# srendle/libfm

Hardware: NVIDIA H100
Metric: MovieLens-1M-shaped examples/sec at k=8, SGD (higher is better)
Workload: dtype f32

## Files before the change

include/fmb200.h:

```cpp
#ifndef FMB200_H_
#define FMB200_H_

#include <stdint.h>

#ifdef __cplusplus
extern "C" {
#endif

typedef struct fmb200_ctx fmb200_ctx;

#define FMB200_TASK_REGRESSION 0
#define FMB200_TASK_CLASSIFICATION 1

#define FMB200_MODE_INORDER 0
#define FMB200_MODE_HOGWILD 1

#define FMB200_MODE_ORDERED 2

#define FMB200_MAX_SLOTS 8
#define FMB200_MAX_PEERS 16
#define FMB200_IPC_HANDLE_BYTES 64

int fmb200_create(fmb200_ctx** out, int device, uint32_t n_attr, int num_factor, int use_w0,
                  int use_w);
void fmb200_destroy(fmb200_ctx* ctx);
const char* fmb200_last_error(void);

int fmb200_set_hparams(fmb200_ctx* ctx, int task, double learn_rate, double reg0, double regw,
                       double regv, double min_target, double max_target);
int fmb200_set_mode(fmb200_ctx* ctx, int mode);

int fmb200_upload_data(fmb200_ctx* ctx, int slot, uint64_t n_rows, uint64_t nnz,
                       const uint64_t* row_ptr, const uint32_t* col, const float* val,
                       const float* target);
int fmb200_upload_data_async(fmb200_ctx* ctx, int slot, uint64_t n_rows, uint64_t nnz,
                             const uint64_t* row_ptr, const uint32_t* col, const float* val,
                             const float* target);
int fmb200_upload_data_aos(fmb200_ctx* ctx, int slot, uint64_t n_rows, const void* rows,
                           const float* target);
int fmb200_upload_onehot(fmb200_ctx* ctx, int slot, uint64_t n_rows, uint32_t nnz_per_row,
                         const uint32_t* ids, const float* target);
int fmb200_upload_onehot_async(fmb200_ctx* ctx, int slot, uint64_t n_rows, uint32_t nnz_per_row,
                               const uint32_t* ids, const float* target);
int fmb200_free_data(fmb200_ctx* ctx, int slot);

int fmb200_host_alloc(void** out, uint64_t bytes);
int fmb200_host_free(void* p);

int fmb200_set_params(fmb200_ctx* ctx, double w0, const double* w, const double* v_factor_major);
int fmb200_get_params(fmb200_ctx* ctx, double* w0, double* w, double* v_factor_major);

int fmb200_sgd_epoch(fmb200_ctx* ctx, int slot, double* device_seconds);
int fmb200_sgd_epoch_async(fmb200_ctx* ctx, int slot);
int fmb200_sync(fmb200_ctx* ctx);

int fmb200_evaluate(fmb200_ctx* ctx, int slot, double* sum_sq_err, double* sum_abs_err,
                    uint64_t* n_correct);

int fmb200_predict(fmb200_ctx* ctx, int slot, int transform, double* out);

int fmb200_mcmc_eterms(fmb200_ctx* ctx, int slot, double* e_out);

int fmb200_mcmc_begin(fmb200_ctx* ctx, int train_slot, int test_slot, int do_sample, int do_multilevel,
                      uint32_t n_groups, const uint32_t* attr_group, const uint32_t* attr_per_group, double reg0,
                      const double* w_lambda, const double* v_lambda);
int fmb200_mcmc_iteration(fmb200_ctx* ctx, double* train_metric, uint32_t* counters);
int fmb200_mcmc_get_hyper(fmb200_ctx* ctx, double* alpha, double* w_mu, double* w_lambda, double* v_mu,
                          double* v_lambda);
int fmb200_mcmc_get_pred(fmb200_ctx* ctx, double* pred_this, double* pred_sum_all, double* pred_sum_all_but5);
int fmb200_mcmc_runs(fmb200_ctx* ctx, uint32_t* n_runs);

int fmb200_sgda_begin(fmb200_ctx* ctx, uint32_t n_groups, const uint32_t* attr_group);
int fmb200_sgda_epoch(fmb200_ctx* ctx, int train_slot, int val_slot, int lambda_steps, double* device_seconds);
int fmb200_sgda_get_reg(fmb200_ctx* ctx, double* reg_w, double* reg_v);

int fmb200_params_device(fmb200_ctx* ctx, void** device_ptr, uint64_t* n_floats);
int fmb200_scale_params(fmb200_ctx* ctx, double factor);
int fmb200_params_layout(fmb200_ctx* ctx, uint64_t* off_w, int* ws, uint64_t* off_v, int* kp);
int fmb200_stream(fmb200_ctx* ctx, void** cuda_stream);

int fmb200_peer_export(fmb200_ctx* ctx, void* handle );
int fmb200_peer_attach_ipc(fmb200_ctx* ctx, int world, int rank, const void* handles );
int fmb200_peer_attach_local(fmb200_ctx* ctx, int world, int rank, fmb200_ctx* const* contexts);
int fmb200_allreduce_mean(fmb200_ctx* ctx);
int fmb200_allreduce_meanfield(fmb200_ctx* ctx);
int fmb200_peer_barrier(fmb200_ctx* ctx);

int fmb200_download_data(fmb200_ctx* ctx, int slot, uint64_t* n_rows, uint64_t* nnz, uint64_t* row_ptr,
                         uint32_t* col, float* val, float* target);
int fmb200_kernel_launches(fmb200_ctx* ctx, uint64_t* count);
int fmb200_last_epoch_config(fmb200_ctx* ctx, int* lanes_per_row, int* slots, int* rows_per_tile,
                             int* grid, int* block, int* smem_bytes, int* damp);
int fmb200_set_tuning(fmb200_ctx* ctx, int ctas_per_sm, int rows_per_tile, int threads, int damp,
                      int variant);
int fmb200_ordered_index(fmb200_ctx* ctx, int slot, uint32_t* link ,
                         uint32_t* rowdep );

#ifdef __cplusplus
}
#endif
#endif
```

libfm_b200/_capi.py:

```python
from __future__ import annotations

import ctypes as C
import os

_HERE = os.path.dirname(os.path.abspath(__file__))
LIB_PATH = os.environ.get("FMB200_LIB") or os.path.join(_HERE, "lib", "libfmb200.so")

_u64p = C.POINTER(C.c_uint64)
_u32p = C.POINTER(C.c_uint32)
_f32p = C.POINTER(C.c_float)
_f64p = C.POINTER(C.c_double)
_intp = C.POINTER(C.c_int)
_ctx = C.c_void_p

SYMBOLS = {
    "fmb200_create": (C.c_int, [C.POINTER(_ctx), C.c_int, C.c_uint32, C.c_int, C.c_int, C.c_int]),
    "fmb200_destroy": (None, [_ctx]),
    "fmb200_last_error": (C.c_char_p, []),
    "fmb200_set_hparams": (C.c_int, [_ctx, C.c_int] + [C.c_double] * 6),
    "fmb200_set_mode": (C.c_int, [_ctx, C.c_int]),
    "fmb200_upload_data": (C.c_int, [_ctx, C.c_int, C.c_uint64, C.c_uint64, _u64p, _u32p, _f32p, _f32p]),
    "fmb200_upload_data_async": (C.c_int, [_ctx, C.c_int, C.c_uint64, C.c_uint64, _u64p, _u32p, _f32p, _f32p]),
    "fmb200_upload_data_aos": (C.c_int, [_ctx, C.c_int, C.c_uint64, C.c_void_p, _f32p]),
    "fmb200_upload_onehot": (C.c_int, [_ctx, C.c_int, C.c_uint64, C.c_uint32, _u32p, _f32p]),
    "fmb200_upload_onehot_async": (C.c_int, [_ctx, C.c_int, C.c_uint64, C.c_uint32, _u32p, _f32p]),
    "fmb200_free_data": (C.c_int, [_ctx, C.c_int]),
    "fmb200_host_alloc": (C.c_int, [C.POINTER(C.c_void_p), C.c_uint64]),
    "fmb200_host_free": (C.c_int, [C.c_void_p]),
    "fmb200_set_params": (C.c_int, [_ctx, C.c_double, _f64p, _f64p]),
    "fmb200_get_params": (C.c_int, [_ctx, _f64p, _f64p, _f64p]),
    "fmb200_sgd_epoch": (C.c_int, [_ctx, C.c_int, _f64p]),
    "fmb200_sgd_epoch_async": (C.c_int, [_ctx, C.c_int]),
    "fmb200_sync": (C.c_int, [_ctx]),
    "fmb200_evaluate": (C.c_int, [_ctx, C.c_int, _f64p, _f64p, _u64p]),
    "fmb200_predict": (C.c_int, [_ctx, C.c_int, C.c_int, _f64p]),
    "fmb200_sgda_begin": (C.c_int, [_ctx, C.c_uint32, _u32p]),
    "fmb200_sgda_epoch": (C.c_int, [_ctx, C.c_int, C.c_int, C.c_int, _f64p]),
    "fmb200_sgda_get_reg": (C.c_int, [_ctx, _f64p, _f64p]),
    "fmb200_mcmc_eterms": (C.c_int, [_ctx, C.c_int, _f64p]),
    "fmb200_mcmc_begin": (C.c_int, [_ctx, C.c_int, C.c_int, C.c_int, C.c_int, C.c_uint32, _u32p, _u32p, C.c_double,
                                    _f64p, _f64p]),
    "fmb200_mcmc_iteration": (C.c_int, [_ctx, _f64p, _u32p]),
    "fmb200_mcmc_get_hyper": (C.c_int, [_ctx] + [_f64p] * 5),
    "fmb200_mcmc_get_pred": (C.c_int, [_ctx] + [_f64p] * 3),
    "fmb200_mcmc_runs": (C.c_int, [_ctx, _u32p]),
    "fmb200_params_device": (C.c_int, [_ctx, C.POINTER(C.c_void_p), _u64p]),
    "fmb200_scale_params": (C.c_int, [_ctx, C.c_double]),
    "fmb200_params_layout": (C.c_int, [_ctx, _u64p, _intp, _u64p, _intp]),
    "fmb200_stream": (C.c_int, [_ctx, C.POINTER(C.c_void_p)]),
    "fmb200_peer_export": (C.c_int, [_ctx, C.c_void_p]),
    "fmb200_peer_attach_ipc": (C.c_int, [_ctx, C.c_int, C.c_int, C.c_void_p]),
    "fmb200_peer_attach_local": (C.c_int, [_ctx, C.c_int, C.c_int, C.POINTER(_ctx)]),
    "fmb200_allreduce_mean": (C.c_int, [_ctx]),
    "fmb200_allreduce_meanfield": (C.c_int, [_ctx]),
    "fmb200_peer_barrier": (C.c_int, [_ctx]),
    "fmb200_download_data": (C.c_int, [_ctx, C.c_int, _u64p, _u64p, _u64p, _u32p, _f32p, _f32p]),
    "fmb200_kernel_launches": (C.c_int, [_ctx, _u64p]),
    "fmb200_last_epoch_config": (C.c_int, [_ctx] + [_intp] * 7),
    "fmb200_set_tuning": (C.c_int, [_ctx, C.c_int, C.c_int, C.c_int, C.c_int, C.c_int]),
    "fmb200_ordered_index": (C.c_int, [_ctx, C.c_int, _u32p, _u32p]),
}

_lib = None


def load() -> C.CDLL:
    global _lib
    if _lib is None:
        if not os.path.exists(LIB_PATH):
            raise ImportError(
                f"{LIB_PATH} is missing: build it with `python -m libfm_b200.build` "
                "(libfm_b200 has no CPU fallback)")
        lib = C.CDLL(LIB_PATH)
        for name, (res, args) in SYMBOLS.items():
            fn = getattr(lib, name)
            fn.restype = res
            fn.argtypes = args
        _lib = lib
    return _lib
```

libfm_b200/build.py:

```python
from __future__ import annotations

import concurrent.futures as cf
import os
import shutil
import subprocess
import sys

HERE = os.path.dirname(os.path.abspath(__file__))
ROOT = os.path.dirname(HERE)
CSRC = os.path.join(HERE, "csrc")
HOST = os.path.join(HERE, "host")
LIBDIR = os.path.join(HERE, "lib")
OBJDIR = os.path.join(ROOT, "build", "obj")
BINDIR = os.path.join(ROOT, "bin")

NVCC = os.environ.get("NVCC") or shutil.which("nvcc") or "/usr/local/cuda/bin/nvcc"
ARCH = ["-gencode", "arch=compute_90a,code=sm_90a"]
COMMON = ["-O3", "-std=c++17", "-lineinfo", "-Xcompiler", "-fPIC", "-Xptxas", "-v",
          "-I", os.path.join(ROOT, "include")]

CU_SOURCES = {
    "fm_context.cu": [],
    "fm_hogwild.cu": [],
    "fm_rowlane.cu": [],
    "fm_peer.cu": [],
    "fm_predict.cu": [],
    "fm_inorder.cu": ["--fmad=false"],
    "fm_ordered.cu": [],
    "fm_upload.cu": [],
    "fm_mcmc.cu": ["--fmad=false"],
}
CU_HEADERS = ["fm_device.cuh", "fm_rowgroup.cuh", "fm_hogwild_common.cuh", "fmb200_internal.h",
              "fm_inorder_wavefront.cuh", "fm_ordered.cuh", "fm_roworder.cuh", "ref_random.h"]


def _newer(target: str, deps: list[str]) -> bool:
    if not os.path.exists(target):
        return True
    t = os.path.getmtime(target)
    return any(os.path.getmtime(d) > t for d in deps)


def _run(cmd: list[str], log: str | None = None) -> None:
    p = subprocess.run(cmd, stdout=subprocess.PIPE, stderr=subprocess.STDOUT, text=True)
    if log:
        with open(log, "w") as f:
            f.write(" ".join(cmd) + "\n" + p.stdout)
    if p.returncode != 0:
        sys.stderr.write(p.stdout)
        raise RuntimeError("build step failed: " + " ".join(cmd))


def lib_path() -> str:
    return os.path.join(LIBDIR, "libfmb200.so")


def cli_path() -> str:
    return os.path.join(BINDIR, "libFM")


def build_lib(force: bool = False) -> str:
    os.makedirs(LIBDIR, exist_ok=True)
    os.makedirs(OBJDIR, exist_ok=True)
    hdrs = [os.path.join(CSRC, h) for h in CU_HEADERS] + [os.path.join(ROOT, "include", "fmb200.h")]
    jobs = []
    objs = []
    for src, extra in CU_SOURCES.items():
        s = os.path.join(CSRC, src)
        o = os.path.join(OBJDIR, src.replace(".cu", ".o"))
        objs.append(o)
        if force or _newer(o, [s] + hdrs):
            cmd = [NVCC, *ARCH, *COMMON, *extra, "-c", s, "-o", o]
            jobs.append((cmd, o + ".log"))
    if jobs:
        with cf.ThreadPoolExecutor(max_workers=min(len(jobs), os.cpu_count() or 2)) as ex:
            list(ex.map(lambda j: _run(*j), jobs))
    out = lib_path()
    if force or jobs or _newer(out, objs):
        _run([NVCC, *ARCH, "-shared", "-o", out, *objs])
    return out


def build_cli(force: bool = False) -> str | None:
    main = os.path.join(HOST, "libfm_main.cpp")
    if not os.path.exists(main):
        return None
    os.makedirs(BINDIR, exist_ok=True)
    hdrs = [os.path.join(HOST, f) for f in os.listdir(HOST) if f.endswith(".h")]
    hdrs.append(os.path.join(CSRC, "ref_random.h"))
    out = cli_path()
    if force or _newer(out, [main] + hdrs + [lib_path()]):
        cmd = ["g++", "-O2", "-std=c++17", "-Wall", "-I", os.path.join(ROOT, "include"), main,
               "-o", out, "-pthread", "-L", LIBDIR, "-lfmb200", "-Wl,-rpath,$ORIGIN/../libfm_b200/lib"]
        nccl = os.environ.get("FMB200_NCCL", "1") == "1" and os.path.exists("/usr/include/nccl.h")
        cuda_inc = "/usr/local/cuda/include"
        if nccl:
            cmd += ["-DFMB200_WITH_NCCL", "-I", cuda_inc, "-lnccl", "-L/usr/local/cuda/lib64", "-lcudart"]
        _run(cmd)
    conv_src = os.path.join(HOST, "convert_main.cpp")
    conv = os.path.join(BINDIR, "convert")
    if os.path.exists(conv_src) and (force or _newer(conv, [conv_src] + hdrs)):
        _run(["g++", "-O2", "-std=c++17", "-Wall", conv_src, "-o", conv, "-pthread"])
    return out


def build_all(force: bool = False) -> None:
    build_lib(force)
    build_cli(force)


if __name__ == "__main__":
    build_all(force="--force" in sys.argv)
    print(lib_path())
```

libfm_b200/csrc/fm_context.cu:

```cuda
#include <cmath>
#include <cstdarg>
#include <cstdio>
#include <algorithm>
#include <cstring>
#include <new>
#include <vector>

#include "fmb200_internal.h"

using namespace fmb;

namespace {

thread_local char g_err[512] = "";

int fail(const char* fmt, ...) {
  va_list ap;
  va_start(ap, fmt);
  vsnprintf(g_err, sizeof(g_err), fmt, ap);
  va_end(ap);
  return 1;
}

#define CK(expr)                                                                      \
  do {                                                                                \
    cudaError_t e__ = (expr);                                                         \
    if (e__ != cudaSuccess)                                                           \
      return fail("%s failed: %s (%s:%d)", #expr, cudaGetErrorString(e__), __FILE__, \
                  __LINE__);                                                          \
  } while (0)

#define NEED_CTX(c) \
  if ((c) == nullptr) return fail("null context")

template <class F>
int guarded(F&& body) {
  try {
    return body();
  } catch (const std::bad_alloc&) {
    return fail("out of host memory");
  } catch (...) {
    return fail("unexpected C++ exception");
  }
}

int bind(fmb200_ctx* c) {
  CK(cudaSetDevice(c->device));
  return 0;
}

int upload_begin(fmb200_ctx* c, int slot, uint64_t n_rows, uint64_t nnz, cudaStream_t st) {
  DataSlot& s = c->slots[slot];
  if (s.pending) {
    CK(cudaEventSynchronize(s.ready.get()));
    s.pending = false;
  }
  if (!(s.row_ptr && s.cap_rows >= n_rows && s.cap_nnz >= nnz)) {
    s = DataSlot();
    CK(alloc(s.row_ptr, n_rows + 1 + kRowSlack));
    CK(alloc(s.target, n_rows + kRowSlack));
    CK(alloc(s.col, nnz + kEntrySlack));
    CK(alloc(s.val, nnz + kEntrySlack));
    CK(alloc(s.feat_cnt, c->n));
    CK(alloc(s.d_flag, 16));
    CK(host_alloc(s.h_flag, 16));
    CK(event_create(s.ready, cudaEventDisableTiming));
    CK(cudaMemsetAsync(s.row_ptr.get(), 0, (n_rows + 1 + kRowSlack) * sizeof(uint64_t), st));
    CK(cudaMemsetAsync(s.target.get(), 0, (n_rows + kRowSlack) * sizeof(float), st));
    CK(cudaMemsetAsync(s.col.get(), 0, (nnz + kEntrySlack) * sizeof(uint32_t), st));
    CK(cudaMemsetAsync(s.val.get(), 0, (nnz + kEntrySlack) * sizeof(float), st));
    s.cap_rows = n_rows;
    s.cap_nnz = nnz;
  }
  s.present = false;
  s.links_ready = false;
  s.upload_gen = ++c->upload_counter;
  s.n_rows = n_rows;
  s.nnz = nnz;
  return 0;
}

int upload_inspect(fmb200_ctx* c, int slot, cudaStream_t st) {
  DataSlot& s = c->slots[slot];
  unsigned int* flag = s.d_flag.get();
  CK(cudaMemsetAsync(flag, 0, 16 * sizeof(unsigned int), st));
  CK(launch_csr_inspect(c, st, s.row_ptr.get(), s.n_rows, s.nnz, flag));
  CK(launch_feature_counts(c, st, s.col.get(), s.nnz, s.feat_cnt.get(), flag + 8, flag + 9));
  CK(cudaMemcpyAsync(s.h_flag.get(), flag, 16 * sizeof(unsigned int), cudaMemcpyDeviceToHost, st));
  CK(cudaEventRecord(s.ready.get(), st));
  s.pending = true;
  return 0;
}

int upload_enqueue(fmb200_ctx* c, int slot, uint64_t n_rows, uint64_t nnz, const uint64_t* row_ptr,
                   const uint32_t* col, const float* val, const float* target, cudaStream_t st) {
  if (upload_begin(c, slot, n_rows, nnz, st)) return 1;
  DataSlot& s = c->slots[slot];
  CK(cudaMemcpyAsync(s.row_ptr.get(), row_ptr, (n_rows + 1) * sizeof(uint64_t), cudaMemcpyHostToDevice, st));
  CK(cudaMemcpyAsync(s.target.get(), target, n_rows * sizeof(float), cudaMemcpyHostToDevice, st));
  CK(cudaMemcpyAsync(s.col.get(), col, nnz * sizeof(uint32_t), cudaMemcpyHostToDevice, st));
  CK(cudaMemcpyAsync(s.val.get(), val, nnz * sizeof(float), cudaMemcpyHostToDevice, st));
  return upload_inspect(c, slot, st);
}

int upload_onehot_enqueue(fmb200_ctx* c, int slot, uint64_t n_rows, uint32_t z, const uint32_t* ids,
                          const float* target, cudaStream_t st) {
  const uint64_t nnz = n_rows * z;
  if (upload_begin(c, slot, n_rows, nnz, st)) return 1;
  DataSlot& s = c->slots[slot];
  CK(cudaMemcpyAsync(s.target.get(), target, n_rows * sizeof(float), cudaMemcpyHostToDevice, st));
  CK(cudaMemcpyAsync(s.col.get(), ids, nnz * sizeof(uint32_t), cudaMemcpyHostToDevice, st));
  CK(launch_onehot_fill(c, st, n_rows, z, s.row_ptr.get(), s.val.get()));
  return upload_inspect(c, slot, st);
}

int upload_finish(fmb200_ctx* c, int slot) {
  DataSlot& s = c->slots[slot];
  if (!s.pending) return 0;
  CK(cudaEventSynchronize(s.ready.get()));
  s.pending = false;
  const unsigned int* h = s.h_flag.get();
  if (h[0] & 1u) return fail("row_ptr[0] must be 0");
  if (h[0] & 2u) return fail("row_ptr is not monotone");
  if (h[0] & 4u) return fail("row_ptr[n_rows] != nnz");
  if (h[0] & 8u) return fail("a row is longer than 2^32-1 entries");
  if (s.nnz > 0 && h[8] >= c->n)
    return fail("feature id %u out of range (num_attribute=%u)", h[8], c->n);
  s.max_row_nnz = h[1];
  for (int i = 0; i < 5; i++) s.tile_span[i] = h[2 + i];
  s.max_feat_cnt = h[9];
  s.present = true;
  return 0;
}

int upload_common(fmb200_ctx* c, int slot, uint64_t n_rows, uint64_t nnz, const uint64_t* row_ptr,
                  const uint32_t* col, const float* val, const float* target) {
  if (upload_enqueue(c, slot, n_rows, nnz, row_ptr, col, val, target, c->stream)) return 1;
  return upload_finish(c, slot);
}

int need_slot(fmb200_ctx* c, int slot) {
  if (slot < 0 || slot >= FMB200_MAX_SLOTS) return fail("slot %d out of range", slot);
  if (c->slots[slot].pending && upload_finish(c, slot)) return 1;
  if (!c->slots[slot].present) return fail("slot %d holds no data", slot);
  return 0;
}

int need_fp64(const fmb200_ctx* c, const char* what) {
  if (c->mode == FMB200_MODE_HOGWILD) return fail("%s", what);
  return 0;
}

template <class F>
int timed(fmb200_ctx* c, double* device_seconds, F&& body) {
  CK(cudaEventRecord(c->ev0.get(), c->stream));
  if (body()) return 1;
  CK(cudaEventRecord(c->ev1.get(), c->stream));
  CK(cudaStreamSynchronize(c->stream));
  if (device_seconds) {
    float ms = 0.f;
    CK(cudaEventElapsedTime(&ms, c->ev0.get(), c->ev1.get()));
    *device_seconds = (double)ms * 1e-3;
  }
  return 0;
}

}

static int create_resources(fmb200_ctx* c, int device, const cudaDeviceProp& prop, uint32_t n_attr,
                            int num_factor, int use_w0, int use_w) {
  c->device = device;
  c->sm_count = prop.multiProcessorCount;
  c->max_smem_optin = (int)prop.sharedMemPerBlockOptin;
  c->n = n_attr;
  c->k = num_factor;
  c->kp = (num_factor + 3) & ~3;
  c->k0 = use_w0 != 0;
  c->k1 = use_w != 0;
  CK(cudaSetDevice(device));
  CK(cudaStreamCreateWithFlags(&c->stream, cudaStreamNonBlocking));
  CK(event_create(c->ev0, cudaEventDefault));
  CK(event_create(c->ev1, cudaEventDefault));
  c->p32.ws = (n_attr <= 131072u) ? 8 : 1;
  const uint64_t n4 = ((uint64_t)n_attr * c->p32.ws + 3) & ~3ull;
  c->p32.off_w = 4;
  c->p32.off_v = 4 + n4;
  c->p32.n_floats = 4 + n4 + (uint64_t)n_attr * c->kp;
  c->p64.off_v = Params64::off_w + (((uint64_t)n_attr + 1) & ~1ull);
  c->p64.n_doubles = c->p64.off_v + (uint64_t)n_attr * num_factor + 2;
  c->comm = CommLayout(c->p32.n_floats, n_attr);
  CK(alloc(c->comm_base, c->comm.total_bytes()));
  CK(cudaMemsetAsync(c->comm_base.get(), 0, c->comm.total_bytes(), c->stream));
  c->p32.base = c->comm.buf(c->comm_base.get(), 0);
  c->peer_base[0] = c->comm_base.get();
  CK(alloc(c->p64_buf, c->p64.n_doubles));
  c->p64.base = c->p64_buf.get();
  CK(cudaMemsetAsync(c->p32.base, 0, c->p32.n_floats * sizeof(float), c->stream));
  CK(cudaMemsetAsync(c->p64.base, 0, c->p64.n_doubles * sizeof(double), c->stream));
  CK(alloc(c->d_sched, 2));
  CK(cudaMemsetAsync(c->d_sched.get(), 0, 2 * sizeof(unsigned int), c->stream));
  CK(alloc(c->d_gbar, 1));
  CK(cudaMemsetAsync(c->d_gbar.get(), 0, sizeof(unsigned int), c->stream));
  CK(alloc(c->d_flag, 16));
  CK(host_alloc(c->h_flag, 16));
  {
    const size_t need = std::max(c->p32.n_floats * sizeof(float), c->p64.n_doubles * sizeof(double));
    if (need <= (64u << 20)) CK(host_alloc(c->h_stage, need));
  }
  CK(cudaStreamSynchronize(c->stream));
  return 0;
}

extern "C" {

const char* fmb200_last_error(void) { return g_err; }

int fmb200_create(fmb200_ctx** out, int device, uint32_t n_attr, int num_factor, int use_w0,
                  int use_w) {
  if (out == nullptr) return fail("null out pointer");
  *out = nullptr;
  if (num_factor < 0) return fail("num_factor must be >= 0");
  int count = 0;
  cudaError_t e = cudaGetDeviceCount(&count);
  if (e != cudaSuccess || count == 0)
    return fail("no CUDA device available (%s): libfmb200 has no CPU path",
                e == cudaSuccess ? "device count 0" : cudaGetErrorString(e));
  if (device < 0 || device >= count) return fail("device %d out of range (count %d)", device, count);
  cudaDeviceProp prop;
  CK(cudaGetDeviceProperties(&prop, device));
  if (prop.major != 9 || prop.minor != 0)
    return fail("device %d is sm_%d%d; this library contains sm_90a code only", device, prop.major,
                prop.minor);
  fmb200_ctx* c = new (std::nothrow) fmb200_ctx();
  if (!c) return fail("out of host memory");
  if (create_resources(c, device, prop, n_attr, num_factor, use_w0, use_w)) {
    fmb200_destroy(c);
    return 1;
  }
  *out = c;
  return 0;
}

void fmb200_destroy(fmb200_ctx* c) {
  if (!c) return;
  cudaSetDevice(c->device);
  if (c->stream) cudaStreamSynchronize(c->stream);
  for (int q = 0; q < FMB200_MAX_PEERS; q++)
    if (c->peer_ipc[q] && c->peer_base[q]) cudaIpcCloseMemHandle(c->peer_base[q]);
  cudaStream_t stream = c->stream, copy_stream = c->copy_stream;
  delete c;
  if (copy_stream) cudaStreamDestroy(copy_stream);
  if (stream) cudaStreamDestroy(stream);
}

int fmb200_set_hparams(fmb200_ctx* c, int task, double learn_rate, double reg0, double regw,
                       double regv, double min_target, double max_target) {
  NEED_CTX(c);
  if (task != FMB200_TASK_REGRESSION && task != FMB200_TASK_CLASSIFICATION)
    return fail("unknown task");
  c->hp.task = task;
  c->hp.lr = learn_rate;
  c->hp.reg0 = reg0;
  c->hp.regw = regw;
  c->hp.regv = regv;
  c->hp.min_target = min_target;
  c->hp.max_target = max_target;
  return 0;
}

int fmb200_set_mode(fmb200_ctx* c, int mode) {
  NEED_CTX(c);
  if (mode != FMB200_MODE_INORDER && mode != FMB200_MODE_HOGWILD && mode != FMB200_MODE_ORDERED)
    return fail("unknown mode %d", mode);
  if (mode == c->mode) return 0;
  if (bind(c)) return 1;
  const bool was64 = c->mode != FMB200_MODE_HOGWILD, is64 = mode != FMB200_MODE_HOGWILD;
  if (is64 && c->k > 256) return fail("num_factor > 256 is not supported in the fp64 modes");
  if (was64 && !is64) {
    CK(launch_p64_to_p32(c));
  } else if (!was64 && is64) {
    CK(launch_p32_to_p64(c));
  }
  CK(cudaStreamSynchronize(c->stream));
  c->mode = mode;
  c->peer_base_valid = false;
  return 0;
}

int fmb200_upload_data(fmb200_ctx* c, int slot, uint64_t n_rows, uint64_t nnz,
                       const uint64_t* row_ptr, const uint32_t* col, const float* val,
                       const float* target) {
  NEED_CTX(c);
  if (slot < 0 || slot >= FMB200_MAX_SLOTS) return fail("slot %d out of range", slot);
  if (!row_ptr || (n_rows && !target) || (nnz && (!col || !val))) return fail("null data pointer");
  if (n_rows > 0xffffffffull) return fail("row count exceeds the reference's uint range");
  if (bind(c)) return 1;
  return upload_common(c, slot, n_rows, nnz, row_ptr, col, val, target);
}

int fmb200_upload_data_async(fmb200_ctx* c, int slot, uint64_t n_rows, uint64_t nnz,
                             const uint64_t* row_ptr, const uint32_t* col, const float* val,
                             const float* target) {
  NEED_CTX(c);
  if (slot < 0 || slot >= FMB200_MAX_SLOTS) return fail("slot %d out of range", slot);
  if (!row_ptr || (n_rows && !target) || (nnz && (!col || !val))) return fail("null data pointer");
  if (n_rows > 0xffffffffull) return fail("row count exceeds the reference's uint range");
  if (bind(c)) return 1;
  if (c->copy_stream == nullptr) CK(cudaStreamCreateWithFlags(&c->copy_stream, cudaStreamNonBlocking));
  return upload_enqueue(c, slot, n_rows, nnz, row_ptr, col, val, target, c->copy_stream);
}

struct AosEntry {
  uint32_t id;
  float value;
};
struct AosRow {
  const AosEntry* data;
  uint32_t size;
};
static_assert(sizeof(AosRow) == 16 && sizeof(AosEntry) == 8, "LP64 layout of sparse_row/sparse_entry");

static int upload_aos_host_gather(fmb200_ctx* c, int slot, uint64_t n_rows, const AosRow* r,
                                  const float* target) {
  return guarded([&]() -> int {
    std::vector<uint64_t> rp(n_rows + 1);
    rp[0] = 0;
    for (uint64_t i = 0; i < n_rows; i++) rp[i + 1] = rp[i] + r[i].size;
    const uint64_t nnz = rp[n_rows];
    std::vector<uint32_t> col(nnz ? nnz : 1);
    std::vector<float> val(nnz ? nnz : 1);
    for (uint64_t i = 0; i < n_rows; i++) {
      const AosEntry* e = r[i].data;
      uint64_t o = rp[i];
      for (uint32_t j = 0; j < r[i].size; j++) {
        col[o + j] = e[j].id;
        val[o + j] = e[j].value;
      }
    }
    return upload_common(c, slot, n_rows, nnz, rp.data(), col.data(), val.data(), target);
  });
}

int fmb200_upload_data_aos(fmb200_ctx* c, int slot, uint64_t n_rows, const void* rows,
                           const float* target) {
  NEED_CTX(c);
  if (slot < 0 || slot >= FMB200_MAX_SLOTS) return fail("slot %d out of range", slot);
  if (n_rows && (!rows || !target)) return fail("null data pointer");
  if (n_rows > 0xffffffffull) return fail("row count exceeds the reference's uint range");
  if (bind(c)) return 1;
  const AosRow* r = static_cast<const AosRow*>(rows);
  uint64_t first = 0;
  while (first < n_rows && r[first].size == 0) first++;
  if (first == n_rows) {
    std::vector<uint64_t> rp;
    try {
      rp.assign(n_rows + 1, 0);
    } catch (const std::bad_alloc&) {
      return fail("out of host memory");
    }
    uint32_t dc = 0;
    float dv = 0.f;
    return upload_common(c, slot, n_rows, 0, rp.data(), &dc, &dv, target);
  }
  const unsigned long long base = (unsigned long long)(uintptr_t)r[first].data;
  cudaStream_t st = c->stream;
  DevPtr<AosRow> d_rows;
  DevPtr<uint64_t> d_rp;
  DevPtr<unsigned long long> d_scr;
  DevPtr<AosEntry> d_ent;
  unsigned int* flag = c->d_flag.get();
  CK(alloc(d_rows, n_rows));
  CK(alloc(d_rp, n_rows + 1));
  CK(alloc(d_scr, aos_scan_tiles(n_rows) + 1));
  CK(cudaMemsetAsync(flag, 0, 16 * sizeof(unsigned int), st));
  CK(cudaMemcpyAsync(d_rows.get(), r, n_rows * sizeof(AosRow), cudaMemcpyHostToDevice, st));
  CK(launch_aos_to_csr(c, st, d_rows.get(), nullptr, n_rows, 0, base, d_scr.get(), d_rp.get(), nullptr, nullptr, flag));
  uint64_t nnz = 0;
  CK(cudaMemcpyAsync(c->h_flag.get(), flag, sizeof(unsigned int), cudaMemcpyDeviceToHost, st));
  CK(cudaMemcpyAsync(&nnz, d_rp.get() + n_rows, sizeof(uint64_t), cudaMemcpyDeviceToHost, st));
  CK(cudaStreamSynchronize(st));
  if (c->h_flag.get()[0] & 1u) return upload_aos_host_gather(c, slot, n_rows, r, target);
  if (upload_begin(c, slot, n_rows, nnz, st)) return 1;
  DataSlot& s = c->slots[slot];
  CK(alloc(d_ent, nnz));
  CK(cudaMemcpyAsync(d_ent.get(), r[first].data, nnz * sizeof(AosEntry), cudaMemcpyHostToDevice, st));
  CK(cudaMemcpyAsync(s.row_ptr.get(), d_rp.get(), (n_rows + 1) * sizeof(uint64_t), cudaMemcpyDeviceToDevice, st));
  CK(cudaMemcpyAsync(s.target.get(), target, n_rows * sizeof(float), cudaMemcpyHostToDevice, st));
  CK(launch_aos_split(c, st, d_ent.get(), nnz, s.col.get(), s.val.get()));
  if (upload_inspect(c, slot, st)) return 1;
  return upload_finish(c, slot);
}

int fmb200_upload_onehot(fmb200_ctx* c, int slot, uint64_t n_rows, uint32_t nnz_per_row,
                         const uint32_t* ids, const float* target) {
  NEED_CTX(c);
  if (slot < 0 || slot >= FMB200_MAX_SLOTS) return fail("slot %d out of range", slot);
  if (n_rows && (!target || (nnz_per_row && !ids))) return fail("null data pointer");
  if (n_rows > 0xffffffffull) return fail("row count exceeds the reference's uint range");
  if (bind(c)) return 1;
  if (upload_onehot_enqueue(c, slot, n_rows, nnz_per_row, ids, target, c->stream)) return 1;
  return upload_finish(c, slot);
}

int fmb200_upload_onehot_async(fmb200_ctx* c, int slot, uint64_t n_rows, uint32_t nnz_per_row,
                               const uint32_t* ids, const float* target) {
  NEED_CTX(c);
  if (slot < 0 || slot >= FMB200_MAX_SLOTS) return fail("slot %d out of range", slot);
  if (n_rows && (!target || (nnz_per_row && !ids))) return fail("null data pointer");
  if (n_rows > 0xffffffffull) return fail("row count exceeds the reference's uint range");
  if (bind(c)) return 1;
  if (c->copy_stream == nullptr) CK(cudaStreamCreateWithFlags(&c->copy_stream, cudaStreamNonBlocking));
  return upload_onehot_enqueue(c, slot, n_rows, nnz_per_row, ids, target, c->copy_stream);
}

int fmb200_host_alloc(void** out, uint64_t bytes) {
  if (!out) return fail("null out pointer");
  *out = nullptr;
  CK(cudaHostAlloc(out, bytes ? bytes : 1, cudaHostAllocDefault));
  return 0;
}

int fmb200_host_free(void* p) {
  if (p) CK(cudaFreeHost(p));
  return 0;
}

int fmb200_free_data(fmb200_ctx* c, int slot) {
  NEED_CTX(c);
  if (slot < 0 || slot >= FMB200_MAX_SLOTS) return fail("slot %d out of range", slot);
  if (bind(c)) return 1;
  CK(cudaStreamSynchronize(c->stream));
  if (c->slots[slot].pending) CK(cudaEventSynchronize(c->slots[slot].ready.get()));
  c->slots[slot] = DataSlot();
  return 0;
}

int fmb200_set_params(fmb200_ctx* c, double w0, const double* w, const double* v) {
  NEED_CTX(c);
  if ((c->n && !w) || ((uint64_t)c->n * c->k && !v)) return fail("null parameter pointer");
  if (bind(c)) return 1;
  return guarded([&]() -> int {
  const uint32_t n = c->n;
    const int k = c->k, kp = c->kp;
    std::vector<double> h64(c->p64.n_doubles);
    h64[0] = w0;
    for (uint32_t i = 0; i < n; i++) h64[Params64::off_w + i] = w[i];
    double* hv = h64.data() + c->p64.off_v;
    for (int f = 0; f < k; f++)
      for (uint32_t i = 0; i < n; i++) hv[(size_t)i * k + f] = v[(size_t)f * n + i];
    std::vector<float> h32(c->p32.n_floats, 0.f);
    h32[0] = (float)w0;
    for (uint32_t i = 0; i < n; i++) h32[c->p32.off_w + (size_t)i * c->p32.ws] = (float)w[i];
    float* hv32 = h32.data() + c->p32.off_v;
    for (int f = 0; f < k; f++)
      for (uint32_t i = 0; i < n; i++) hv32[(size_t)i * kp + f] = (float)v[(size_t)f * n + i];
    CK(cudaMemcpyAsync(c->p64.base, h64.data(), h64.size() * sizeof(double), cudaMemcpyHostToDevice, c->stream));
    CK(cudaMemcpyAsync(c->p32.base, h32.data(), h32.size() * sizeof(float), cudaMemcpyHostToDevice, c->stream));
    CK(clear_acc_flag(c));
    CK(cudaStreamSynchronize(c->stream));
    c->peer_base_valid = false;
    c->hogwild_fresh = true;
    return 0;
  });
}

int fmb200_get_params(fmb200_ctx* c, double* w0, double* w, double* v) {
  NEED_CTX(c);
  if (!w0 || (c->n && !w) || ((uint64_t)c->n * c->k && !v)) return fail("null parameter pointer");
  if (bind(c)) return 1;
  return guarded([&]() -> int {
  const uint32_t n = c->n;
    const int k = c->k, kp = c->kp;
    if (c->mode != FMB200_MODE_HOGWILD) {
      std::vector<double> pageable;
      double* h = reinterpret_cast<double*>(c->h_stage.get());
      if (h == nullptr) {
        pageable.resize(c->p64.n_doubles);
        h = pageable.data();
      }
      CK(cudaMemcpyAsync(h, c->p64.base, c->p64.n_doubles * sizeof(double), cudaMemcpyDeviceToHost, c->stream));
      CK(cudaStreamSynchronize(c->stream));
      *w0 = h[0];
      for (uint32_t i = 0; i < n; i++) w[i] = h[Params64::off_w + i];
      const double* hv = h + c->p64.off_v;
      for (int f = 0; f < k; f++)
        for (uint32_t i = 0; i < n; i++) v[(size_t)f * n + i] = hv[(size_t)i * k + f];
    } else {
      std::vector<float> pageable;
      float* h = reinterpret_cast<float*>(c->h_stage.get());
      if (h == nullptr) {
        pageable.resize(c->p32.n_floats);
        h = pageable.data();
      }
      CK(cudaMemcpyAsync(h, c->p32.base, c->p32.n_floats * sizeof(float), cudaMemcpyDeviceToHost, c->stream));
      CK(cudaStreamSynchronize(c->stream));
      *w0 = h[0];
      for (uint32_t i = 0; i < n; i++) w[i] = h[c->p32.off_w + (size_t)i * c->p32.ws];
      const float* hv = h + c->p32.off_v;
      for (uint32_t i = 0; i < n; i++)
        for (int f = 0; f < k; f++) v[(size_t)f * n + i] = hv[(size_t)i * kp + f];
    }
    return 0;
  });
}

int fmb200_sgd_epoch_async(fmb200_ctx* c, int slot) {
  NEED_CTX(c);
  if (need_slot(c, slot)) return 1;
  if (bind(c)) return 1;
  DataSlot& d = c->slots[slot];
  if (c->mode == FMB200_MODE_ORDERED) {
    bool handled = false;
    CK(launch_sgd_ordered(c, d, &handled));
    if (!handled) CK(launch_sgd_inorder(c, d));
  } else if (c->mode == FMB200_MODE_INORDER) {
    CK(launch_sgd_inorder(c, d));
  } else {
    if (c->kp > 128) return fail("num_factor > 128 is not supported in HOGWILD mode");
    CK(peer_before_epoch(c, d));
    CK(launch_sgd_hogwild(c, d));
  }
  return 0;
}

int fmb200_sync(fmb200_ctx* c) {
  NEED_CTX(c);
  if (bind(c)) return 1;
  CK(cudaStreamSynchronize(c->stream));
  return 0;
}

int fmb200_sgd_epoch(fmb200_ctx* c, int slot, double* device_seconds) {
  NEED_CTX(c);
  if (bind(c)) return 1;
  return timed(c, device_seconds, [&] { return fmb200_sgd_epoch_async(c, slot); });
}

int fmb200_evaluate(fmb200_ctx* c, int slot, double* sum_sq_err, double* sum_abs_err,
                    uint64_t* n_correct) {
  NEED_CTX(c);
  if (need_slot(c, slot)) return 1;
  if (bind(c)) return 1;
  const DataSlot& d = c->slots[slot];
  double sq = 0, ab = 0, ok = 0;
  if (d.n_rows > 0) {
    const int nb = grid_for(c, d.n_rows);
    CK(grow(c->d_partials, c->n_partials, 3 * (uint64_t)nb));
    if (c->mode != FMB200_MODE_HOGWILD && c->hp.task == FMB200_TASK_REGRESSION) {
      CK(grow(c->d_pred, c->pred_cap, d.n_rows));
      CK(launch_predict64(c, d, 2, c->d_pred.get(), nullptr, nb));
      std::vector<double> err;
      try {
        err.resize(d.n_rows);
      } catch (const std::bad_alloc&) {
        return fail("out of host memory");
      }
      CK(cudaMemcpyAsync(err.data(), c->d_pred.get(), d.n_rows * sizeof(double), cudaMemcpyDeviceToHost, c->stream));
      CK(cudaStreamSynchronize(c->stream));
      for (uint64_t i = 0; i < d.n_rows; i++) {
        sq += err[i] * err[i];
        ab += std::abs(err[i]);
      }
    } else {
      if (c->mode != FMB200_MODE_HOGWILD) {
        CK(launch_predict64(c, d, 0, nullptr, c->d_partials.get(), nb));
      } else {
        CK(launch_predict32(c, d, 0, nullptr, c->d_partials.get(), nb));
      }
      std::vector<double> h;
      try {
        h.resize(3 * (size_t)nb);
      } catch (const std::bad_alloc&) {
        return fail("out of host memory");
      }
      CK(cudaMemcpyAsync(h.data(), c->d_partials.get(), h.size() * sizeof(double), cudaMemcpyDeviceToHost, c->stream));
      CK(cudaStreamSynchronize(c->stream));
      for (int b = 0; b < nb; b++) {
        sq += h[3 * b + 0];
        ab += h[3 * b + 1];
        ok += h[3 * b + 2];
      }
    }
  }
  if (sum_sq_err) *sum_sq_err = sq;
  if (sum_abs_err) *sum_abs_err = ab;
  if (n_correct) *n_correct = (uint64_t)llround(ok);
  return 0;
}

int fmb200_predict(fmb200_ctx* c, int slot, int transform, double* out) {
  NEED_CTX(c);
  if (need_slot(c, slot)) return 1;
  if (bind(c)) return 1;
  const DataSlot& d = c->slots[slot];
  if (d.n_rows == 0) return 0;
  if (!out) return fail("null output pointer");
  CK(grow(c->d_pred, c->pred_cap, d.n_rows));
  const int nb = grid_for(c, d.n_rows);
  if (c->mode != FMB200_MODE_HOGWILD) {
    CK(launch_predict64(c, d, transform, c->d_pred.get(), nullptr, nb));
  } else {
    CK(launch_predict32(c, d, transform, c->d_pred.get(), nullptr, nb));
  }
  CK(cudaMemcpyAsync(out, c->d_pred.get(), d.n_rows * sizeof(double), cudaMemcpyDeviceToHost, c->stream));
  CK(cudaStreamSynchronize(c->stream));
  return 0;
}

int fmb200_sgda_begin(fmb200_ctx* c, uint32_t n_groups, const uint32_t* attr_group) {
  NEED_CTX(c);
  if (bind(c)) return 1;
  if (need_fp64(c, "SGDA runs on the fp64 state: set INORDER or ORDERED mode first")) return 1;
  if (n_groups == 0 || n_groups > 1024) return fail("n_groups must be in [1,1024]");
  if (n_groups > 1 && !attr_group) return fail("attr_group is required for more than one group");
  if (attr_group)
    for (uint32_t i = 0; i < c->n; i++)
      if (attr_group[i] >= n_groups) return fail("attr_group[%u] = %u >= n_groups", i, attr_group[i]);
  const size_t n1 = c->n ? c->n : 1, nk = (size_t)c->n * c->k ? (size_t)c->n * c->k : 1;
  const size_t gk = (size_t)n_groups * (c->k ? c->k : 1);
  if (!c->sgda_grad_w) {
    CK(alloc(c->sgda_grad_w, n1));
    CK(alloc(c->sgda_grad_v, nk));
    CK(alloc(c->sgda_group, n1));
  }
  if (c->sgda_groups != n_groups) {
    c->sgda_groups = 0;
    CK(alloc(c->sgda_reg_w, n_groups));
    CK(alloc(c->sgda_reg_v, gk));
    c->sgda_groups = n_groups;
  }
  CK(cudaMemsetAsync(c->sgda_grad_w.get(), 0, n1 * sizeof(double), c->stream));
  CK(cudaMemsetAsync(c->sgda_grad_v.get(), 0, nk * sizeof(double), c->stream));
  CK(cudaMemsetAsync(c->sgda_reg_w.get(), 0, n_groups * sizeof(double), c->stream));
  CK(cudaMemsetAsync(c->sgda_reg_v.get(), 0, gk * sizeof(double), c->stream));
  CK(cudaMemsetAsync(c->p64.w(), 0, n1 * sizeof(double), c->stream));
  if (attr_group) CK(cudaMemcpyAsync(c->sgda_group.get(), attr_group, c->n * sizeof(uint32_t), cudaMemcpyHostToDevice, c->stream));
  else CK(cudaMemsetAsync(c->sgda_group.get(), 0, n1 * sizeof(uint32_t), c->stream));
  CK(cudaStreamSynchronize(c->stream));
  return 0;
}

int fmb200_sgda_epoch(fmb200_ctx* c, int train_slot, int val_slot, int lambda_steps, double* device_seconds) {
  NEED_CTX(c);
  if (need_slot(c, train_slot) || need_slot(c, val_slot)) return 1;
  if (bind(c)) return 1;
  if (need_fp64(c, "SGDA runs on the fp64 state: set INORDER or ORDERED mode first")) return 1;
  if (c->sgda_groups == 0) return fail("call fmb200_sgda_begin first");
  return timed(c, device_seconds, [&]() -> int {
    CK(launch_sgda_epoch(c, c->slots[train_slot], c->slots[val_slot], lambda_steps));
    return 0;
  });
}

int fmb200_sgda_get_reg(fmb200_ctx* c, double* reg_w, double* reg_v) {
  NEED_CTX(c);
  if (bind(c)) return 1;
  if (c->sgda_groups == 0) return fail("call fmb200_sgda_begin first");
  if (reg_w) CK(cudaMemcpyAsync(reg_w, c->sgda_reg_w.get(), c->sgda_groups * sizeof(double), cudaMemcpyDeviceToHost, c->stream));
  if (reg_v && c->k)
    CK(cudaMemcpyAsync(reg_v, c->sgda_reg_v.get(), (size_t)c->sgda_groups * c->k * sizeof(double), cudaMemcpyDeviceToHost, c->stream));
  CK(cudaStreamSynchronize(c->stream));
  return 0;
}

int fmb200_mcmc_eterms(fmb200_ctx* c, int slot, double* e_out) {
  NEED_CTX(c);
  if (need_slot(c, slot)) return 1;
  if (bind(c)) return 1;
  if (need_fp64(c, "e-terms are computed from the fp64 state: set INORDER or ORDERED mode first")) return 1;
  const DataSlot& d = c->slots[slot];
  if (d.n_rows == 0) return 0;
  if (!e_out) return fail("null output pointer");
  CK(grow(c->d_pred, c->pred_cap, d.n_rows));
  CK(launch_mcmc_eterms(c, d, c->d_pred.get()));
  CK(cudaMemcpyAsync(e_out, c->d_pred.get(), d.n_rows * sizeof(double), cudaMemcpyDeviceToHost, c->stream));
  CK(cudaStreamSynchronize(c->stream));
  return 0;
}

int fmb200_mcmc_begin(fmb200_ctx* c, int train_slot, int test_slot, int do_sample, int do_multilevel,
                      uint32_t n_groups, const uint32_t* attr_group, const uint32_t* attr_per_group, double reg0,
                      const double* w_lambda, const double* v_lambda) {
  NEED_CTX(c);
  if (need_slot(c, train_slot) || need_slot(c, test_slot)) return 1;
  if (bind(c)) return 1;
  if (need_fp64(c, "MCMC / ALS run on the fp64 state: set INORDER or ORDERED mode first")) return 1;
  if (!w_lambda || (!v_lambda && c->k > 0)) return fail("null w_lambda / v_lambda");
  if (c->peer_world > 1) return fail("MCMC / ALS run on one GPU: this context is attached to a multi-GPU peer world");
  return guarded([&]() {
    const std::string e = mcmc_begin(c, train_slot, test_slot, do_sample, do_multilevel, n_groups, attr_group,
                                      attr_per_group, reg0, w_lambda, v_lambda);
    if (!e.empty()) {
      c->mcmc.reset();
      return fail("fmb200_mcmc_begin: %s", e.c_str());
    }
    return 0;
  });
}

int fmb200_mcmc_iteration(fmb200_ctx* c, double* train_metric, uint32_t* counters) {
  NEED_CTX(c);
  if (!c->mcmc) return fail("call fmb200_mcmc_begin first");
  if (need_fp64(c, "MCMC / ALS run on the fp64 state: set INORDER or ORDERED mode first")) return 1;
  if (bind(c)) return 1;
  return guarded([&]() {
    double m = 0.0;
    const std::string e = mcmc_iteration(c, &m, counters);
    if (!e.empty()) return fail("fmb200_mcmc_iteration: %s", e.c_str());
    if (train_metric) *train_metric = m;
    return 0;
  });
}

int fmb200_mcmc_get_hyper(fmb200_ctx* c, double* alpha, double* w_mu, double* w_lambda, double* v_mu,
                          double* v_lambda) {
  NEED_CTX(c);
  if (!mcmc_get(c, alpha, w_mu, w_lambda, v_mu, v_lambda, nullptr, nullptr, nullptr, nullptr))
    return fail("call fmb200_mcmc_begin first");
  return 0;
}

int fmb200_mcmc_get_pred(fmb200_ctx* c, double* pred_this, double* pred_sum_all, double* pred_sum_all_but5) {
  NEED_CTX(c);
  if (!mcmc_get(c, nullptr, nullptr, nullptr, nullptr, nullptr, pred_this, pred_sum_all, pred_sum_all_but5, nullptr))
    return fail("call fmb200_mcmc_begin first");
  return 0;
}

int fmb200_mcmc_runs(fmb200_ctx* c, uint32_t* n_runs) {
  NEED_CTX(c);
  if (!mcmc_get(c, nullptr, nullptr, nullptr, nullptr, nullptr, nullptr, nullptr, nullptr, n_runs))
    return fail("call fmb200_mcmc_begin first");
  return 0;
}

int fmb200_params_device(fmb200_ctx* c, void** device_ptr, uint64_t* n_floats) {
  NEED_CTX(c);
  if (c->mode != FMB200_MODE_HOGWILD) return fail("packed fp32 state is live only in HOGWILD mode");
  if (device_ptr) *device_ptr = c->p32.base;
  if (n_floats) *n_floats = c->p32.n_floats;
  return 0;
}

int fmb200_params_layout(fmb200_ctx* c, uint64_t* off_w, int* ws, uint64_t* off_v, int* kp) {
  NEED_CTX(c);
  if (off_w) *off_w = c->p32.off_w;
  if (ws) *ws = c->p32.ws;
  if (off_v) *off_v = c->p32.off_v;
  if (kp) *kp = c->kp;
  return 0;
}

int fmb200_scale_params(fmb200_ctx* c, double factor) {
  NEED_CTX(c);
  if (c->mode != FMB200_MODE_HOGWILD) return fail("scale_params applies to the HOGWILD state");
  if (bind(c)) return 1;
  CK(launch_scale_p32(c, (float)factor));
  c->peer_base_valid = false;
  return 0;
}

int fmb200_peer_export(fmb200_ctx* c, void* handle) {
  NEED_CTX(c);
  if (!handle) return fail("null handle pointer");
  if (bind(c)) return 1;
  static_assert(sizeof(cudaIpcMemHandle_t) == FMB200_IPC_HANDLE_BYTES, "IPC handle size");
  cudaIpcMemHandle_t h;
  CK(cudaIpcGetMemHandle(&h, c->comm_base.get()));
  memcpy(handle, &h, sizeof(h));
  return 0;
}

static int peer_precheck(fmb200_ctx* c, int world, int rank) {
  if (world < 1 || world > FMB200_MAX_PEERS) return fail("world %d outside [1,%d]", world, FMB200_MAX_PEERS);
  if (rank < 0 || rank >= world) return fail("rank %d outside world %d", rank, world);
  if (c->peer_seq != 0 || c->peer_world != 1) return fail("peers are already attached");
  if (c->mode != FMB200_MODE_HOGWILD) return fail("peer averaging applies to the HOGWILD state");
  return 0;
}

int fmb200_peer_attach_ipc(fmb200_ctx* c, int world, int rank, const void* handles) {
  NEED_CTX(c);
  if (!handles) return fail("null handles");
  if (peer_precheck(c, world, rank)) return 1;
  if (bind(c)) return 1;
  const unsigned char* hb = static_cast<const unsigned char*>(handles);
  for (int q = 0; q < world; q++) {
    if (q == rank) {
      c->peer_base[q] = c->comm_base.get();
      continue;
    }
    cudaIpcMemHandle_t h;
    memcpy(&h, hb + (size_t)q * FMB200_IPC_HANDLE_BYTES, sizeof(h));
    void* p = nullptr;
    CK(cudaIpcOpenMemHandle(&p, h, cudaIpcMemLazyEnablePeerAccess));
    c->peer_base[q] = static_cast<unsigned char*>(p);
    c->peer_ipc[q] = true;
  }
  CK(peer_preload_kernels());
  c->peer_world = world;
  c->peer_rank = rank;
  return 0;
}

int fmb200_peer_attach_local(fmb200_ctx* c, int world, int rank, fmb200_ctx* const* all) {
  NEED_CTX(c);
  if (!all) return fail("null context list");
  if (peer_precheck(c, world, rank)) return 1;
  if (bind(c)) return 1;
  for (int q = 0; q < world; q++) {
    if (!all[q] || all[q]->p32.n_floats != c->p32.n_floats) return fail("peer %d has a different model shape", q);
    if (q != rank && all[q]->device != c->device) {
      int can = 0;
      CK(cudaDeviceCanAccessPeer(&can, c->device, all[q]->device));
      if (!can) return fail("device %d cannot access device %d", c->device, all[q]->device);
      cudaError_t e = cudaDeviceEnablePeerAccess(all[q]->device, 0);
      if (e != cudaSuccess && e != cudaErrorPeerAccessAlreadyEnabled)
        return fail("cudaDeviceEnablePeerAccess failed: %s", cudaGetErrorString(e));
      (void)cudaGetLastError();
    }
    c->peer_base[q] = all[q]->comm_base.get();
  }
  CK(peer_preload_kernels());
  c->peer_world = world;
  c->peer_rank = rank;
  return 0;
}

int fmb200_allreduce_mean(fmb200_ctx* c) {
  NEED_CTX(c);
  if (c->mode != FMB200_MODE_HOGWILD) return fail("peer averaging applies to the HOGWILD state");
  if (c->peer_world <= 1) return 0;
  if (bind(c)) return 1;
  CK(launch_peer_mean(c));
  return 0;
}

int fmb200_allreduce_meanfield(fmb200_ctx* c) {
  NEED_CTX(c);
  if (c->mode != FMB200_MODE_HOGWILD) return fail("the peer exchange applies to the HOGWILD state");
  if (c->peer_world <= 1) return 0;
  if (!c->peer_base_valid) return fail("no epoch has run since the state was last set: nothing to combine");
  if (bind(c)) return 1;
  CK(launch_peer_meanfield(c));
  return 0;
}

int fmb200_peer_barrier(fmb200_ctx* c) {
  NEED_CTX(c);
  if (c->peer_world <= 1) return 0;
  if (bind(c)) return 1;
  CK(launch_peer_barrier(c));
  return 0;
}

int fmb200_stream(fmb200_ctx* c, void** cuda_stream) {
  NEED_CTX(c);
  if (cuda_stream) *cuda_stream = (void*)c->stream;
  return 0;
}

int fmb200_kernel_launches(fmb200_ctx* c, uint64_t* count) {
  NEED_CTX(c);
  if (count) *count = c->launches;
  return 0;
}

int fmb200_last_epoch_config(fmb200_ctx* c, int* lanes_per_row, int* slots, int* rows_per_tile,
                             int* grid, int* block, int* smem_bytes, int* damp) {
  NEED_CTX(c);
  if (lanes_per_row) *lanes_per_row = c->last_cfg.lanes_per_row;
  if (slots) *slots = c->last_cfg.slots;
  if (rows_per_tile) *rows_per_tile = c->last_cfg.rows_per_tile;
  if (grid) *grid = c->last_cfg.grid;
  if (block) *block = c->last_cfg.block;
  if (smem_bytes) *smem_bytes = c->last_cfg.smem;
  if (damp) *damp = c->last_cfg.damp;
  return 0;
}

int fmb200_download_data(fmb200_ctx* c, int slot, uint64_t* n_rows, uint64_t* nnz, uint64_t* row_ptr,
                         uint32_t* col, float* val, float* target) {
  NEED_CTX(c);
  if (need_slot(c, slot)) return 1;
  if (bind(c)) return 1;
  const DataSlot& d = c->slots[slot];
  if (n_rows) *n_rows = d.n_rows;
  if (nnz) *nnz = d.nnz;
  if (row_ptr) CK(cudaMemcpyAsync(row_ptr, d.row_ptr.get(), (d.n_rows + 1) * sizeof(uint64_t), cudaMemcpyDeviceToHost, c->stream));
  if (col && d.nnz) CK(cudaMemcpyAsync(col, d.col.get(), d.nnz * sizeof(uint32_t), cudaMemcpyDeviceToHost, c->stream));
  if (val && d.nnz) CK(cudaMemcpyAsync(val, d.val.get(), d.nnz * sizeof(float), cudaMemcpyDeviceToHost, c->stream));
  if (target && d.n_rows) CK(cudaMemcpyAsync(target, d.target.get(), d.n_rows * sizeof(float), cudaMemcpyDeviceToHost, c->stream));
  CK(cudaStreamSynchronize(c->stream));
  return 0;
}

int fmb200_ordered_index(fmb200_ctx* c, int slot, uint32_t* link, uint32_t* rowdep) {
  NEED_CTX(c);
  if (need_slot(c, slot)) return 1;
  if (bind(c)) return 1;
  DataSlot& d = c->slots[slot];
  if (d.nnz >= 0xffffffffull) return fail("the ORDERED index needs nnz < 2^32-1");
  CK(build_ordered_links(c, d));
  if (link && d.nnz)
    CK(cudaMemcpyAsync(link, d.link.get(), d.nnz * sizeof(uint32_t), cudaMemcpyDeviceToHost, c->stream));
  if (rowdep && d.n_rows)
    CK(cudaMemcpyAsync(rowdep, d.rowdep.get(), d.n_rows * sizeof(uint32_t), cudaMemcpyDeviceToHost, c->stream));
  CK(cudaStreamSynchronize(c->stream));
  return 0;
}

int fmb200_set_tuning(fmb200_ctx* c, int ctas_per_sm, int rows_per_tile, int threads, int damp,
                      int variant) {
  NEED_CTX(c);
  if (threads && (threads % 32 != 0 || threads < 32 || threads > 1024))
    return fail("threads must be a multiple of 32 in [32,1024]");
  if (rows_per_tile && (rows_per_tile < 32 || rows_per_tile > 512))
    return fail("rows_per_tile must be in [32,512]");
  c->tune_ctas_per_sm = ctas_per_sm;
  c->tune_rows_per_tile = rows_per_tile;
  c->tune_threads = threads;
  c->tune_damp = damp;
  c->tune_variant = variant;
  return 0;
}

}
```

libfm_b200/csrc/fm_hogwild.cu:

```cuda
#include <algorithm>
#include <cstdio>

#include "fm_hogwild_common.cuh"
#include "fm_rowgroup.cuh"

namespace fmb {

template <int G, int S, int R, int RW, int U, bool DAMP>
__global__ void __launch_bounds__(HW_MAX_THREADS, (R * U <= 4 ? 3 : (R > 20 ? 1 : 2)))
    fm_sgd_hogwild_kernel(const HogwildArgs a) {
  using RG = RowGroup<G, S, R, RW>;
  constexpr int E = RG::E;
  constexpr int RPW = 32 / E;
  extern __shared__ __align__(128) unsigned char smem[];
  uint64_t* bars = reinterpret_cast<uint64_t*>(smem);
  float* s_acc = reinterpret_cast<float*>(smem + 64);

  const int tid = threadIdx.x;
  const int lane = tid & 31;
  const int warp = tid >> 5;
  const int nwarp = blockDim.x >> 5;
  const int rows_per_set = nwarp * RPW;
  const int lig = lane % E;
  const int c = lig % G;
  const int s = lig / G;
  const int sub = lane / E;
  const int TR = a.tile_rows;

  const uint64_t policy = ring_init(smem, tid);
  uint32_t* s_tile = reinterpret_cast<uint32_t*>(smem + 208);
  TileSched sched{a.sched, a.n_tiles, false};
  const int ptid = (int)blockDim.x - 32;
  uint32_t claim_raw = HW_NO_TILE;
  if (tid == ptid) {
    for (int i = 0; i < HW_NSTAGE; i++) {
      const uint32_t t = sched.claim();
      s_tile[i] = t;
      if (t != HW_NO_TILE) {
        const uint64_t r0 = (uint64_t)t * TR, r1 = min(r0 + (uint64_t)TR, a.n_rows);
        issue_tile(a, smem, bars, t, i, policy, __ldg(a.row_ptr + r0), __ldg(a.row_ptr + r1));
      }
    }
    claim_raw = sched.fire();
  }
  __syncthreads();

  const float4* V4 = reinterpret_cast<const float4*>(a.v);
  const bool use_w = a.use_w != 0;
  const bool use_w0 = a.use_w0 != 0;
  const float lr = a.lr;
  const float nlr_regv = -lr * a.regv;
  const float nlr_regw = -lr * a.regw;

  int it = 0;
  for (;; ++it) {
    const int stage = it % HW_NSTAGE;
    const uint32_t parity = (uint32_t)(it / HW_NSTAGE) & 1u;
    const uint64_t tile = s_tile[stage];
    if (tile == HW_NO_TILE) break;
    uint32_t nt = HW_NO_TILE;
    uint64_t nt_nb = 0, nt_ne = 0;
    if (tid == ptid) {
      nt = sched.resolve(claim_raw);
      claim_raw = sched.fire();
      if (nt != HW_NO_TILE) {
        const uint64_t r0 = (uint64_t)nt * TR, r1 = min(r0 + (uint64_t)TR, a.n_rows);
        nt_nb = __ldg(a.row_ptr + r0);
        nt_ne = __ldg(a.row_ptr + r1);
      }
    }
    BiasFetch bias;
    bias.slot = reinterpret_cast<float*>(smem + 192);
    bias.issue(a, use_w0, tid);
    mbar_wait(bars + stage, parity);

    unsigned char* sb = stage_base(smem, a, stage);
    const uint64_t* rp = reinterpret_cast<const uint64_t*>(sb);
    const float* ys = reinterpret_cast<const float*>(sb + (size_t)(TR + 2) * 8);
    const uint32_t* ids = reinterpret_cast<const uint32_t*>(sb + (size_t)(TR + 2) * 8 + (size_t)TR * 4);
    const float* xs = reinterpret_cast<const float*>(ids + a.tile_cap);
    const uint64_t row0 = tile * (uint64_t)TR;
    const int rows_here = (int)min((uint64_t)TR, a.n_rows - row0);
    const uint64_t ab = rp[0] & ~3ull;
    if (a.global_entries) {
      ids = a.col + ab;
      xs = a.val + ab;
    }

    float msum = 0.f, hsum = 0.f;
    float w0 = 0.f;
    bool have_w0 = false;
    for (int rbase = warp * RPW; rbase < rows_here; rbase += U * rows_per_set) {
      RG g[U];
      float y[U];
      bool valid[U];
#pragma unroll
      for (int u = 0; u < U; ++u) {
        const int r = rbase + u * rows_per_set + sub;
        valid[u] = r < rows_here;
        int beg = 0, end = 0;
        y[u] = 0.f;
        if (valid[u]) {
          beg = (int)(rp[r] - ab);
          end = (int)(rp[r + 1] - ab);
          y[u] = ys[r];
        }
        g[u].gather(V4, a.w, a.gp, a.ws, use_w, ids, xs, beg, end, c, s, lig);
      }
      if (!have_w0) {
        w0 = bias.get(use_w0, tid, it, (int)blockDim.x);
        have_w0 = true;
      }
#pragma unroll
      for (int u = 0; u < U; ++u) {
        if (U > 1 && rbase + u * rows_per_set >= rows_here) break;
        RG& gu = g[u];
        const float part = gu.template reduce<DAMP>(V4, a.w, a.gp, a.ws, use_w, ids, xs, c, s, lig);
        const LossStep ls = loss_step(a, w0 + part, y[u]);
        const float mult = ls.mult, curv = ls.curv;
        const float hjoint = DAMP ? curv * ((use_w0 ? 1.f : 0.f) + gu.hrow) : curv;
        if (valid[u] && lig == 0) {
          msum += mult;
          hsum += hjoint;
        }

        const float nlr_mult = -lr * mult;
        auto update_v = [&](int j, const float4& v) {
          const uint32_t id = ids[j];
          const float x = xs[j];
          const float x2 = x * x;
          float sv = 1.f;
          if (DAMP) {
            const float conc = __ldg(a.feat_cnt + id) * a.conc_scale;
            if (conc > 1.f) sv = gamma_scale(conc, lr * (hjoint + a.regv));
          }
          red_add_f4(a.v + ((size_t)id * a.gp + c) * 4,
                     sv * (nlr_mult * (gu.acc.x * x - v.x * x2) + nlr_regv * v.x),
                     sv * (nlr_mult * (gu.acc.y * x - v.y * x2) + nlr_regv * v.y),
                     sv * (nlr_mult * (gu.acc.z * x - v.z * x2) + nlr_regv * v.z),
                     sv * (nlr_mult * (gu.acc.w * x - v.w * x2) + nlr_regv * v.w));
        };
        if (c < a.gp) {
#pragma unroll
          for (int q = 0; q < R; ++q) {
            const int j = gu.beg + s + q * S;
            if (j < gu.end) update_v(j, gu.vc[q]);
          }
          for (int q = R; q < gu.maxit; ++q) {
            const int j = gu.beg + s + q * S;
            if (j < gu.end) update_v(j, ld_cg_f4(V4 + (size_t)ids[j] * a.gp + c));
          }
        }
        auto update_w = [&](int j, float wv) {
          const uint32_t id = ids[j];
          const float x = xs[j];
          float sw = 1.f;
          if (DAMP) {
            const float conc = __ldg(a.feat_cnt + id) * a.conc_scale;
            if (conc > 1.f) sw = gamma_scale(conc, lr * (hjoint + a.regw));
          }
          red_add_f(a.w + (size_t)id * a.ws, sw * (nlr_mult * x + nlr_regw * wv));
        };
        if (use_w) {
#pragma unroll
          for (int t = 0; t < RW; ++t) {
            const int j = gu.beg + lig + t * E;
            if (j < gu.end) update_w(j, gu.wc[t]);
          }
          for (int t = RW; t < gu.maxwit; ++t) {
            const int j = gu.beg + lig + t * E;
            if (j < gu.end) update_w(j, ld_cg_f(a.w + (size_t)ids[j] * a.ws));
          }
        }
      }
    }

    if (!have_w0) w0 = bias.get(use_w0, tid, it, (int)blockDim.x);
    float2* s_part = reinterpret_cast<float2*>(s_acc) + (it & 1) * 8;
    if (use_w0) bias_partial(s_part, msum, hsum, tid);
    __syncthreads();
    if (tid == ptid) {
      s_tile[stage] = nt;
      if (nt != HW_NO_TILE) issue_tile(a, smem, bars, nt, stage, policy, nt_nb, nt_ne);
      if (use_w0) {
        float M = 0.f, H = 0.f;
        for (int i = 0; i < nwarp; i++) {
          M += s_part[i].x;
          H += s_part[i].y;
        }
        const float T = (float)rows_here;
        M += T * a.reg0 * w0;
        const float gsc = gamma_scale(fmaxf(a.w0_conc, 1.f), lr * (H / T + a.reg0));
        red_add_f(a.w0, -lr * gsc * M);
      }
    }
  }
  if (tid == ptid) sched.finish(gridDim.x, claim_raw);
}

using KernelFn = HogwildKernelFn;

template <int G, int S, int R, int RW, int U>
KernelFn pick_damp(bool damp) {
  return damp ? fm_sgd_hogwild_kernel<G, S, R, RW, U, true>
              : fm_sgd_hogwild_kernel<G, S, R, RW, U, false>;
}

template <int G, int S>
KernelFn pick_r(int cls, bool damp) {
  switch (cls) {
    case -1: return pick_damp<G, S, 1, 1, 4>(damp);
    case 0: return pick_damp<G, S, 2, 1, 2>(damp);
    case 1: return pick_damp<G, S, 8, 2, 1>(damp);
    case 2: return pick_damp<G, S, 20, 2, 1>(damp);
    default:
      if constexpr (G == 32) return pick_damp<G, S, 40, 2, 1>(damp);
      else return pick_damp<G, S, 20, 2, 1>(damp);
  }
}

template <int G>
KernelFn pick_s(int S, int R, bool damp) {
  if constexpr (G <= 4) {
    if (S >= 8) return pick_r<G, 8>(R, damp);
  }
  if constexpr (G <= 8) {
    if (S >= 4) return pick_r<G, 4>(R, damp);
  }
  if constexpr (G <= 16) {
    if (S >= 2) return pick_r<G, 2>(R, damp);
  }
  return pick_r<G, 1>(R, damp);
}

static KernelFn pick_kernel(int G, int S, int R, bool damp) {
  switch (G) {
    case 1: return pick_s<1>(S, R, damp);
    case 2: return pick_s<2>(S, R, damp);
    case 4: return pick_s<4>(S, R, damp);
    case 8: return pick_s<8>(S, R, damp);
    case 16: return pick_s<16>(S, R, damp);
    default: return pick_s<32>(S, R, damp);
  }
}

void pick_geometry(int kp, uint64_t n_rows, uint64_t nnz, int* G, int* S, int* cls) {
  int gp = kp / 4;
  int g = 1;
  while (g < gp) g <<= 1;
  if (g > 32) g = 32;
  double avg = n_rows ? (double)nnz / (double)n_rows : 1.0;
  int s = 1;
  while (s < avg && s < 8) s <<= 1;
  while (g * s > 32) s >>= 1;
  if (s < 1) s = 1;
  *G = g;
  *S = s;
  const int iters = (int)((avg + s - 1) / s);
  *cls = iters <= 1 ? -1 : (iters <= 2 ? 0 : (iters <= 8 ? 1 : ((iters <= 20 || g < 32) ? 2 : 3)));
}

static bool want_damp(const fmb200_ctx* c, const DataSlot& d, double flight_per_sm) {
  const double flight_guess = std::min<double>((double)d.n_rows, (double)c->sm_count * flight_per_sm);
  const double q_max = (double)d.max_feat_cnt * flight_guess / (double)d.n_rows * c->hp.lr *
                       (1.0 + std::max(c->hp.regw, c->hp.regv));
  return c->tune_damp == 1 || (c->tune_damp == 0 && q_max > 0.5);
}

static cudaError_t fit_grid(fmb200_ctx* c, HogwildKernelFn fn, int threads, int smem, uint64_t n_tiles,
                            int* grid) {
  cudaError_t e = cudaFuncSetAttribute(fn, cudaFuncAttributeMaxDynamicSharedMemorySize, smem);
  if (e != cudaSuccess) return e;
  int occ = 0;
  e = cudaOccupancyMaxActiveBlocksPerMultiprocessor(&occ, fn, threads, smem);
  if (e != cudaSuccess) return e;
  if (occ < 1) return cudaErrorInvalidConfiguration;
  const int per_sm = c->tune_ctas_per_sm > 0 ? std::min(c->tune_ctas_per_sm, occ) : occ;
  *grid = (int)std::min<uint64_t>(n_tiles, (uint64_t)c->sm_count * per_sm);
  return cudaSuccess;
}

static HogwildArgs make_args(fmb200_ctx* c, const DataSlot& d, uint64_t n_tiles, int TR,
                             uint32_t tile_cap, uint32_t sbytes) {
  HogwildArgs a;
  a.row_ptr = d.row_ptr.get();
  a.col = d.col.get();
  a.val = d.val.get();
  a.target = d.target.get();
  a.n_rows = d.n_rows;
  a.n_tiles = (uint32_t)n_tiles;
  a.tile_rows = TR;
  a.tile_cap = tile_cap;
  a.stage_bytes = sbytes;
  a.w0 = c->p32.w0();
  a.w = c->p32.w();
  a.v = c->p32.v();
  a.gp = c->kp / 4;
  a.ws = c->p32.ws;
  a.use_w0 = c->k0;
  a.use_w = c->k1;
  a.task = c->hp.task;
  a.lr = (float)c->hp.lr;
  a.reg0 = (float)c->hp.reg0;
  a.regw = (float)c->hp.regw;
  a.regv = (float)c->hp.regv;
  a.min_target = (float)c->hp.min_target;
  a.max_target = (float)c->hp.max_target;
  a.feat_cnt = d.feat_cnt.get();
  a.conc_scale = 1.f;
  a.w0_conc = 1.f;
  a.acc_w0 = a.acc_w = a.acc_v = a.acc_bad = a.acc = nullptr;
  a.state = nullptr;
  a.n_acc = 0;
  a.ramp_tiles = 0;
  a.ramp_conc_scale = a.ramp_w0_conc = 1.f;
  a.gbar = nullptr;
  a.gbar_base = 0;
  a.prof = nullptr;
  a.sched = c->d_sched.get();
  a.global_entries = 0;
  return a;
}

static unsigned long long* acc_flag(fmb200_ctx* c) { return c->d_acc.get() + c->p32.n_floats; }

cudaError_t clear_acc_flag(fmb200_ctx* c) {
  return c->d_acc ? cudaMemsetAsync(acc_flag(c), 0, sizeof(unsigned long long), c->stream) : cudaSuccess;
}

static cudaError_t launch_rowlane(fmb200_ctx* c, const DataSlot& d, bool* handled) {
  *handled = false;
  const int gp = c->kp / 4;
  if (gp < 1 || gp > 2 || d.max_row_nnz > 4 || c->tune_variant == 1) return cudaSuccess;
  int threads = c->tune_threads > 0 ? std::min(c->tune_threads, HW_MAX_THREADS) : 256;
  int tr_idx = 0;
  while ((32 << (tr_idx + 1)) <= threads) tr_idx++;
  threads = 32 << tr_idx;
  const int TR = threads;
  const uint32_t cap = (d.tile_span[tr_idx] + 3u) & ~3u;
  const uint32_t sbytes = (uint32_t)hw_stage_bytes(TR, cap);
  const bool damp = want_damp(c, d, 3.0 * TR);
  const bool combine = (double)d.max_feat_cnt * 32.0 / (double)d.n_rows > 0.5;
  const bool ws = c->tune_variant == 3;
  const bool want_prof = c->tune_variant == 132;
  HogwildKernelFn fn = ws ? pick_rowlane_ws_kernel(gp, (int)d.max_row_nnz, damp, combine)
                          : pick_rowlane_kernel(gp, (int)d.max_row_nnz, damp, combine, want_prof);
  if (fn == nullptr) return cudaSuccess;
  const int smem = (ws ? HW_WS_HDR_BYTES : HW_HDR_BYTES) + HW_NSTAGE * (int)sbytes;
  const int launch_threads = ws ? threads + 32 : threads;
  const uint64_t n_tiles = (d.n_rows + TR - 1) / TR;
  int grid = 0;
  cudaError_t e = fit_grid(c, fn, launch_threads, smem, n_tiles, &grid);
  if (e != cudaSuccess) return e;
  HogwildArgs a = make_args(c, d, n_tiles, TR, cap, sbytes);
  a.conc_scale = (float)(std::min<double>((double)d.n_rows, (double)grid * TR) / (double)d.n_rows);
  a.w0_conc = (float)std::min<double>((double)d.n_rows, (double)grid * TR * (ws ? HW_NSTAGE : 1));
  constexpr uint64_t kRampTiles = 4;
  const bool ramp = c->hogwild_fresh && c->k0 && c->tune_damp >= 0 && n_tiles > 8 * kRampTiles;
  c->hogwild_fresh = false;
  if (ws) {
    if (ramp) {
      HogwildArgs r = a;
      r.n_rows = kRampTiles * (uint64_t)TR;
      r.n_tiles = (uint32_t)kRampTiles;
      r.conc_scale = (float)((double)TR / (double)d.n_rows);
      r.w0_conc = (float)TR;
      fn<<<1, launch_threads, smem, c->stream>>>(r);
      c->launches++;
      const uint64_t skip = kRampTiles * (uint64_t)TR;
      a.row_ptr += skip;
      a.target += skip;
      a.n_rows -= skip;
      a.n_tiles = (uint32_t)(n_tiles - kRampTiles);
    }
    fn<<<grid, launch_threads, smem, c->stream>>>(a);
    c->launches++;
  } else {
    const uint64_t n_acc = c->p32.n_floats;
    if (n_acc % 4 != 0) return cudaErrorInvalidValue;
    if (!c->d_acc) {
      if ((e = alloc(c->d_acc, n_acc + 1)) != cudaSuccess) return e;
      e = cudaMemsetAsync(c->d_acc.get(), 0, (n_acc + 1) * sizeof(unsigned long long), c->stream);
      if (e != cudaSuccess) return e;
    }
    unsigned long long* acc = c->d_acc.get();
    float* base = c->p32.base;
    a.acc_w0 = acc + (a.w0 - base);
    a.acc_w = acc + (a.w - base);
    a.acc_v = acc + (a.v - base);
    a.acc_bad = acc_flag(c);
    a.state = base;
    a.acc = acc;
    a.n_acc = n_acc;
    if (ramp) {
      a.ramp_tiles = (uint32_t)kRampTiles;
      a.ramp_conc_scale = (float)((double)TR / (double)d.n_rows);
      a.ramp_w0_conc = (float)TR;
    }
    a.gbar = c->d_gbar.get();
    a.gbar_base = c->gbar_count;
    if (want_prof) {
      if ((e = cudaMalloc(&a.prof, RL_PROF_SLOTS * sizeof(unsigned long long))) != cudaSuccess) return e;
      if ((e = cudaMemsetAsync(a.prof, 0, RL_PROF_SLOTS * sizeof(unsigned long long), c->stream)) != cudaSuccess)
        return e;
    }
    void* args[] = {&a};
    e = cudaLaunchCooperativeKernel((const void*)fn, dim3(grid), dim3(launch_threads), args, (size_t)smem,
                                    c->stream);
    if (e != cudaSuccess) {
      cudaFree(a.prof);
      return e;
    }
    c->launches++;
    const uint32_t n_win = rowlane_windows(a.n_tiles, a.ramp_tiles, (uint32_t)grid);
    c->gbar_count += (uint32_t)grid * rowlane_barriers(a.n_tiles, a.ramp_tiles, (uint32_t)grid);
    if (want_prof) {
      unsigned long long h[RL_PROF_SLOTS];
      if ((e = cudaMemcpyAsync(h, a.prof, sizeof(h), cudaMemcpyDeviceToHost, c->stream)) != cudaSuccess) return e;
      if ((e = cudaStreamSynchronize(c->stream)) != cudaSuccess) return e;
      cudaFree(a.prof);
      static const char* name[RL_PROF_SLOTS] = {"bias+gather", "score+issue", "bulk_wait", "barrier1", "fold",
                                                "barrier2"};
      fprintf(stderr, "[rowlane phases, cycles per window of CTA thread 0 (%u windows x %d CTAs)]", n_win, grid);
      for (int i = 0; i < RL_PROF_SLOTS; i++) fprintf(stderr, " %s=%.1f", name[i], (double)h[i] / n_win / grid);
      fprintf(stderr, "\n");
    }
  }
  c->last_cfg = EpochConfig{1, (int)std::max<uint32_t>(1, d.max_row_nnz), TR, grid, launch_threads, smem, damp ? 1 : 0};
  *handled = true;
  return cudaGetLastError();
}

cudaError_t launch_sgd_hogwild(fmb200_ctx* c, const DataSlot& d) {
  if (c->kp / 4 > 32) return cudaErrorInvalidValue;
  if (d.n_rows == 0) return cudaSuccess;
  {
    bool handled = false;
    cudaError_t e = launch_rowlane(c, d, &handled);
    if (e != cudaSuccess || handled) return e;
  }
  int G, S, cls;
  pick_geometry(c->kp, d.n_rows, d.nnz, &G, &S, &cls);
  const int R = cls < 0 ? 1 : (cls == 0 ? 2 : (cls == 1 ? 8 : (cls == 2 ? 20 : 40)));
  const int U = cls < 0 ? 4 : (cls == 0 ? 2 : 1);
  const int threads = c->tune_threads > 0 ? std::min(c->tune_threads, HW_MAX_THREADS) : 256;
  const int ctas_target = (R * U <= 4) ? 3 : (R > 20 ? 1 : 2);

  const int budget = (c->max_smem_optin - 1024) / ctas_target;
  int tr_idx = 3;
  if (c->tune_rows_per_tile > 0) {
    tr_idx = 0;
    while (tr_idx < 4 && (32 << (tr_idx + 1)) <= c->tune_rows_per_tile) tr_idx++;
  }
  auto stage_bytes_for = [&](int idx) {
    return hw_stage_bytes(32 << idx, ((uint64_t)d.tile_span[idx] + 3u) & ~3ull);
  };
  while (tr_idx > 0 && (uint64_t)HW_HDR_BYTES + HW_NSTAGE * stage_bytes_for(tr_idx) > (uint64_t)budget) tr_idx--;
  const bool global_entries =
      (uint64_t)HW_HDR_BYTES + (uint64_t)HW_NSTAGE * stage_bytes_for(tr_idx) > (uint64_t)c->max_smem_optin;
  if (global_entries) tr_idx = 1;
  const int TR = 32 << tr_idx;
  const uint32_t cap = global_entries ? 0u : (d.tile_span[tr_idx] + 3u) & ~3u;
  const uint32_t sbytes = (uint32_t)hw_stage_bytes(TR, cap);
  const int smem = HW_HDR_BYTES + HW_NSTAGE * (int)sbytes;

  const double rows_per_cta_step = (double)(threads / 32) * (32.0 / (G * S)) * U;
  const bool damp = want_damp(c, d, ctas_target * rows_per_cta_step);

  KernelFn fn = pick_kernel(G, S, cls, damp);
  const uint64_t n_tiles = (d.n_rows + TR - 1) / TR;
  int grid = 0;
  cudaError_t e = fit_grid(c, fn, threads, smem, n_tiles, &grid);
  if (e != cudaSuccess) return e;

  HogwildArgs a = make_args(c, d, n_tiles, TR, cap, sbytes);
  a.global_entries = global_entries ? 1 : 0;
  a.conc_scale = (float)(std::min<double>((double)d.n_rows, (double)grid * rows_per_cta_step) /
                         (double)d.n_rows);
  a.w0_conc = (float)std::min<double>((double)d.n_rows, (double)grid * TR);
  fn<<<grid, threads, smem, c->stream>>>(a);
  c->launches++;
  c->last_cfg = EpochConfig{G, S, TR, grid, threads, smem, damp ? 1 : 0};
  return cudaGetLastError();
}

}
```

libfm_b200/csrc/fm_hogwild_common.cuh:

```cuda
#pragma once
#include "fm_device.cuh"
#include "fmb200_internal.h"

namespace fmb {

constexpr int HW_NSTAGE = 3;
constexpr int HW_MAX_THREADS = 256;
constexpr uint32_t HW_NO_TILE = 0xffffffffu;
constexpr int HW_HDR_BYTES = 256;
constexpr int HW_WS_HDR_BYTES = 512;

template <typename T>
__host__ __device__ inline T hw_rp_bytes(int TR) { return (T)(TR + 2) * 8; }
template <typename T>
__host__ __device__ inline T hw_y_bytes(int TR) { return (T)TR * 4; }
__host__ __device__ inline uint64_t hw_stage_bytes(int TR, uint64_t cap) {
  return (hw_rp_bytes<uint64_t>(TR) + hw_y_bytes<uint64_t>(TR) + 2 * cap * 4 + 15) & ~15ull;
}

struct HogwildArgs {
  const uint64_t* row_ptr;
  const uint32_t* col;
  const float* val;
  const float* target;
  uint64_t n_rows;
  uint32_t n_tiles;
  int tile_rows;
  uint32_t tile_cap;
  uint32_t stage_bytes;
  float* w0;
  float* w;
  float* v;
  int gp;
  int ws;
  int use_w0, use_w, task;
  float lr, reg0, regw, regv, min_target, max_target;
  const float* feat_cnt;
  float conc_scale;
  float w0_conc;
  unsigned int* sched;
  int global_entries;
  unsigned long long *acc_w0, *acc_w, *acc_v;
  unsigned long long* acc_bad;
  float* state;
  unsigned long long* acc;
  uint64_t n_acc;
  uint32_t ramp_tiles;
  float ramp_conc_scale, ramp_w0_conc;
  unsigned int* gbar;
  uint32_t gbar_base;
  unsigned long long* prof;
};

__host__ __device__ inline uint32_t rowlane_windows(uint32_t n_tiles, uint32_t ramp, uint32_t G) {
  return ramp + (n_tiles - ramp + G - 1) / G;
}
__host__ __device__ inline uint32_t rowlane_barriers(uint32_t n_tiles, uint32_t ramp, uint32_t G) {
  return 2u * rowlane_windows(n_tiles, ramp, G) - 1u;
}

struct GridBarrier {
  unsigned int* count;
  uint32_t target;
  __device__ __forceinline__ void arrive(int tid) {
    __syncthreads();
    if (tid == 0) red_release_add_u32(count, 1u);
    target += gridDim.x;
  }
  __device__ __forceinline__ void wait(int tid) {
    if (tid == 0)
      while ((int32_t)(ld_acquire_u32(count) - target) < 0) {
      }
    __syncthreads();
  }
};

constexpr float kAccScale = 0x1p32f;
constexpr float kAccStepMax = 0x1p11f;

__device__ __forceinline__ void acc_add(unsigned long long* p, float d, unsigned long long* bad) {
  if (fabsf(d) < kAccStepMax) red_add_u64(p, (unsigned long long)__float2ll_rn(d * kAccScale));
  else atomicOr(bad, 1ull);
}
__device__ __forceinline__ unsigned long long acc_quantise(float d, unsigned long long* bad) {
  if (fabsf(d) < kAccStepMax) return (unsigned long long)__float2ll_rn(d * kAccScale);
  atomicOr(bad, 1ull);
  return 0ull;
}

__device__ __forceinline__ unsigned char* stage_base(unsigned char* smem, const HogwildArgs& a,
                                                     int stage, int hdr = HW_HDR_BYTES) {
  return smem + hdr + (size_t)stage * a.stage_bytes;
}

__device__ __forceinline__ void issue_tile(const HogwildArgs& a, unsigned char* smem, uint64_t* bars,
                                           uint32_t tile, int stage, uint64_t policy, uint64_t nb,
                                           uint64_t ne, int hdr = HW_HDR_BYTES) {
  const int TR = a.tile_rows;
  const uint64_t r0 = (uint64_t)tile * TR;
  const uint64_t ab = nb & ~3ull;
  const uint64_t ae = (ne + 3ull) & ~3ull;
  const uint32_t ebytes = a.global_entries ? 0u : (uint32_t)(ae - ab) * 4u;
  const uint32_t rp_bytes = hw_rp_bytes<uint32_t>(TR);
  const uint32_t y_bytes = hw_y_bytes<uint32_t>(TR);
  unsigned char* sb = stage_base(smem, a, stage, hdr);
  uint64_t* bar = bars + stage;
  mbar_arrive_expect_tx(bar, rp_bytes + y_bytes + 2u * ebytes);
  bulk_g2s_hint(sb, a.row_ptr + r0, rp_bytes, bar, policy);
  bulk_g2s_hint(sb + rp_bytes, a.target + r0, y_bytes, bar, policy);
  if (ebytes) {
    unsigned char* cb = sb + rp_bytes + y_bytes;
    bulk_g2s_hint(cb, a.col + ab, ebytes, bar, policy);
    bulk_g2s_hint(cb + (size_t)a.tile_cap * 4u, a.val + ab, ebytes, bar, policy);
  }
}

__device__ __forceinline__ uint64_t ring_init(unsigned char* smem, int tid) {
  uint64_t* bars = reinterpret_cast<uint64_t*>(smem);
  uint64_t policy = 0;
  if (tid == 0) {
    for (int i = 0; i < HW_NSTAGE; i++) mbar_init(bars + i, 1);
    fence_mbar_init();
  }
  if (tid == (int)blockDim.x - 32) policy = policy_evict_first();
  __syncthreads();
  return policy;
}

struct LossStep {
  float mult, curv;
};
__device__ __forceinline__ LossStep loss_step(const HogwildArgs& a, float p, float y) {
  LossStep l;
  if (a.task == FMB200_TASK_REGRESSION) {
    const float pc = fmaxf(a.min_target, fminf(a.max_target, p));
    l.mult = pc - y;
    const float den = p - y;
    l.curv = (pc == p) ? 1.f : (fabsf(den) > 1e-12f ? fminf(fmaxf(l.mult / den, 0.f), 1.f) : 0.f);
  } else {
    const float sg = 1.f / (1.f + __expf(-y * p));
    l.mult = -y * (1.f - sg);
    l.curv = sg * (1.f - sg);
  }
  return l;
}

__device__ __forceinline__ float gamma_scale(float c, float u) {
  if (c <= 1.f || u <= 0.f) return 1.f;
  const float q = c * u;
  if (q < 1e-3f) return 1.f;
  const float a = fmaxf(1.f - u, 0.f);
  const float ac = a > 0.f ? __expf(c * __logf(a)) : 0.f;
  return fminf(1.f, (1.f - ac) / q);
}

__device__ __forceinline__ void bias_partial(float2* part, float mult, float hjoint, int tid) {
  mult = warp_sum(mult);
  hjoint = warp_sum(hjoint);
  if ((tid & 31) == 0) part[tid >> 5] = make_float2(mult, hjoint);
}

struct BiasFetch {
  float* slot;
  float pending;
  __device__ __forceinline__ void issue(const HogwildArgs& a, bool use_w0, int tid) {
    pending = 0.f;
    if (use_w0 && tid == 0) pending = ld_cg_f(a.w0);
  }
  __device__ __forceinline__ float get(bool use_w0, int tid, int it, int nthreads) {
    if (!use_w0) return 0.f;
    float* s = slot + (it & 1);
    if (tid < 32) {
      const float v = __shfl_sync(0xffffffffu, pending, 0);
      if (tid == 0) *s = v;
      __threadfence_block();
      named_bar_arrive(1, nthreads);
      return v;
    }
    named_bar_sync(1, nthreads);
    return *s;
  }
};

struct TileSched {
  unsigned int* w;
  uint32_t n_tiles;
  bool dry;
  __device__ __forceinline__ uint32_t claim() {
    if (dry) return HW_NO_TILE;
    const uint32_t t = atomicAdd(w, 1u);
    if (t >= n_tiles) {
      dry = true;
      return HW_NO_TILE;
    }
    return t;
  }
  __device__ __forceinline__ uint32_t fire() { return dry ? HW_NO_TILE : atomicAdd(w, 1u); }
  __device__ __forceinline__ uint32_t resolve(uint32_t raw) {
    if (raw >= n_tiles) {
      dry = true;
      return HW_NO_TILE;
    }
    return raw;
  }
  __device__ __forceinline__ void finish(unsigned int n_ctas, uint32_t last_raw) {
    unsigned int inc = (last_raw == 0x7fffffffu) ? 2u : 1u;
    __threadfence();
    if (atomicAdd(w + 1, inc) == n_ctas - 1) {
      w[0] = 0u;
      w[1] = 0u;
    }
  }
};

using HogwildKernelFn = void (*)(const HogwildArgs);

HogwildKernelFn pick_rowlane_kernel(int gp, int max_row_nnz, bool damp, bool combine, bool prof);
constexpr int RL_PROF_SLOTS = 6;
HogwildKernelFn pick_rowlane_ws_kernel(int gp, int max_row_nnz, bool damp, bool combine);

}
```

libfm_b200/csrc/fm_rowlane.cu:

```cuda
#include <algorithm>

#include "fm_hogwild_common.cuh"

namespace fmb {

template <int GP>
struct FactorRow {
  float v[4 * GP];
};

template <int GP, int Z>
__device__ __forceinline__ void acc_add_row(unsigned long long* acc_v, uint32_t id, bool live,
                                            const float (&d)[4 * GP], int e, int tid, unsigned long long* bad) {
  constexpr int K = 4 * GP;
  __shared__ __align__(128) unsigned long long s_wb[2][HW_MAX_THREADS][K];
  unsigned long long* slot = s_wb[e & 1][tid];
  bulk_wait_read<Z == 1 ? 0 : 1>();
  if (live) {
#pragma unroll
    for (int f = 0; f < K; f += 2)
      *reinterpret_cast<ulonglong2*>(slot + f) = make_ulonglong2(acc_quantise(d[f], bad), acc_quantise(d[f + 1], bad));
    fence_proxy_async_shared();
    bulk_red_add_u64(acc_v + (size_t)id * K, slot, K * 8);
  }
  bulk_commit();
}

template <int GP, int Z, bool DAMP, bool COMBINE, bool ACC, typename W0F>
__device__ __forceinline__ void rowlane_tile(const HogwildArgs& a, const uint64_t* rp,
                                             const float* ys, const uint32_t* ids,
                                             const float* xs, int rows_here, int tid, W0F get_w0,
                                             float& mult_out, float& hjoint_out) {
  constexpr int K = 4 * GP;
  const int lane = tid & 31;
  const int odd = lane & 1;
  const float4* V4 = reinterpret_cast<const float4*>(a.v);
  const bool use_w = a.use_w != 0;
  const bool use_w0 = a.use_w0 != 0;
  const float lr = a.lr;
  const uint64_t ab = rp[0] & ~3ull;
  const bool valid = tid < rows_here;
  int beg = 0, cnt = 0;
  float y = 0.f;
  if (valid) {
    beg = (int)(rp[tid] - ab);
    cnt = (int)(rp[tid + 1] - ab) - beg;
    y = ys[tid];
  }
  uint32_t id[Z];
  float x[Z], wv[Z];
  FactorRow<GP> vr[Z];
#pragma unroll
  for (int e = 0; e < Z; ++e) {
    const bool on = e < cnt;
    id[e] = on ? ids[beg + e] : 0u;
    x[e] = on ? xs[beg + e] : 0.f;
  }
#pragma unroll
  for (int e = 0; e < Z; ++e) {
    if (GP == 2) {
      const uint32_t gid = (e < cnt) ? id[e] : 0xffffffffu;
      const uint32_t pid = __shfl_xor_sync(0xffffffffu, gid, 1);
      const uint32_t idA = odd ? pid : gid;
      const uint32_t idB = odd ? gid : pid;
      const float4 zero4 = make_float4(0.f, 0.f, 0.f, 0.f);
      const float4 la = idA != 0xffffffffu ? ld_cg_f4(V4 + (size_t)idA * 2 + odd) : zero4;
      const float4 lb = idB != 0xffffffffu ? ld_cg_f4(V4 + (size_t)idB * 2 + odd) : zero4;
      const float4 send = odd ? la : lb;
      float4 recv;
      recv.x = __shfl_xor_sync(0xffffffffu, send.x, 1);
      recv.y = __shfl_xor_sync(0xffffffffu, send.y, 1);
      recv.z = __shfl_xor_sync(0xffffffffu, send.z, 1);
      recv.w = __shfl_xor_sync(0xffffffffu, send.w, 1);
      const float4 lo = odd ? recv : la;
      const float4 hi = odd ? lb : recv;
      vr[e].v[0] = lo.x; vr[e].v[1] = lo.y; vr[e].v[2] = lo.z; vr[e].v[3] = lo.w;
      vr[e].v[4] = hi.x; vr[e].v[5] = hi.y; vr[e].v[6] = hi.z; vr[e].v[7] = hi.w;
    } else {
      const float4 l = (e < cnt) ? ld_cg_f4(V4 + (size_t)id[e]) : make_float4(0.f, 0.f, 0.f, 0.f);
      vr[e].v[0] = l.x; vr[e].v[1] = l.y; vr[e].v[2] = l.z; vr[e].v[3] = l.w;
    }
    wv[e] = (use_w && e < cnt) ? ld_cg_f(a.w + (size_t)id[e] * a.ws) : 0.f;
  }

  float sum[K];
#pragma unroll
  for (int f = 0; f < K; ++f) sum[f] = 0.f;
  float sq = 0.f, lin = 0.f, xx = 0.f;
#pragma unroll
  for (int e = 0; e < Z; ++e) {
#pragma unroll
    for (int f = 0; f < K; ++f) {
      const float d = vr[e].v[f] * x[e];
      sum[f] += d;
      sq += d * d;
    }
    lin += wv[e] * x[e];
    xx += x[e] * x[e];
  }
  float s2 = 0.f;
#pragma unroll
  for (int f = 0; f < K; ++f) s2 += sum[f] * sum[f];
  const float w0 = get_w0();
  const float p = w0 + lin + 0.5f * (s2 - sq);

  const LossStep ls = loss_step(a, p, y);
  float mult = ls.mult, curv = ls.curv;
  if (!valid) {
    mult = 0.f;
    curv = 0.f;
  }
  const float hrow = (use_w ? xx : 0.f) + fmaxf((xx - 2.f) * s2 + sq, 0.f);
  const float hjoint = DAMP ? curv * ((use_w0 ? 1.f : 0.f) + hrow) : curv;

  const float nlr_mult = -lr * mult;
  const float nlr_regv = -lr * a.regv;
  const float nlr_regw = -lr * a.regw;
#pragma unroll
  for (int e = 0; e < Z; ++e) {
    const bool on = e < cnt;
    float sv = 1.f, sw = 1.f;
    if (DAMP) {
      const float conc = on ? __ldg(a.feat_cnt + id[e]) * a.conc_scale : 0.f;
      if (conc > 1.f) {
        sv = gamma_scale(conc, lr * (hjoint + a.regv));
        sw = gamma_scale(conc, lr * (hjoint + a.regw));
      }
    }
    const float x2 = x[e] * x[e];
    float d[K];
#pragma unroll
    for (int f = 0; f < K; ++f)
      d[f] = sv * (nlr_mult * (sum[f] * x[e] - vr[e].v[f] * x2) + nlr_regv * vr[e].v[f]);
    float dw = sw * (nlr_mult * x[e] + nlr_regw * wv[e]);
    bool on_c = on;
    if (COMBINE) {
      const uint32_t key = on ? id[e] : (0x80000000u | (uint32_t)lane);
      unsigned peers = __match_any_sync(0xffffffffu, key);
      if (__any_sync(0xffffffffu, __popc(peers) > 1)) {
        const int first = __ffs(peers) - 1;
        int rel = __popc(peers << (31 - lane) << 1);
        peers &= (0xfffffffeu << lane);
        while (__any_sync(0xffffffffu, peers != 0u)) {
          const int next = __ffs(peers);
          const int src = next ? next - 1 : lane;
#pragma unroll
          for (int f = 0; f < K; ++f) {
            const float t = __shfl_sync(0xffffffffu, d[f], src);
            if (next) d[f] += t;
          }
          const float tw = __shfl_sync(0xffffffffu, dw, src);
          if (next) dw += tw;
          const unsigned done = __ballot_sync(0xffffffffu, rel & 1);
          peers &= ~done;
          rel >>= 1;
        }
        on_c = on && (lane == first);
      }
    }
    if constexpr (ACC) {
      acc_add_row<GP, Z>(a.acc_v, id[e], on_c, d, e, tid, a.acc_bad);
    } else if (GP == 2) {
      const uint32_t pid = __shfl_xor_sync(0xffffffffu, id[e], 1);
      const bool pon = __shfl_xor_sync(0xffffffffu, (int)on_c, 1) != 0;
      const uint32_t idA = odd ? pid : id[e];
      const uint32_t idB = odd ? id[e] : pid;
      const bool onA = odd ? pon : on_c;
      const bool onB = odd ? on_c : pon;
      float4 send, keep;
      if (odd) {
        send = make_float4(d[0], d[1], d[2], d[3]);
        keep = make_float4(d[4], d[5], d[6], d[7]);
      } else {
        send = make_float4(d[4], d[5], d[6], d[7]);
        keep = make_float4(d[0], d[1], d[2], d[3]);
      }
      float4 recv;
      recv.x = __shfl_xor_sync(0xffffffffu, send.x, 1);
      recv.y = __shfl_xor_sync(0xffffffffu, send.y, 1);
      recv.z = __shfl_xor_sync(0xffffffffu, send.z, 1);
      recv.w = __shfl_xor_sync(0xffffffffu, send.w, 1);
      const float4 va = odd ? recv : keep;
      const float4 vb = odd ? keep : recv;
      if (onA) red_add_f4(a.v + ((size_t)idA * 2 + odd) * 4, va.x, va.y, va.z, va.w);
      if (onB) red_add_f4(a.v + ((size_t)idB * 2 + odd) * 4, vb.x, vb.y, vb.z, vb.w);
    } else if (on_c) {
      red_add_f4(a.v + (size_t)id[e] * 4, d[0], d[1], d[2], d[3]);
    }
    if (on_c && use_w) {
      if (ACC) acc_add(a.acc_w + (size_t)id[e] * a.ws, dw, a.acc_bad);
      else red_add_f(a.w + (size_t)id[e] * a.ws, dw);
    }
  }

  mult_out = mult;
  hjoint_out = valid ? hjoint : 0.f;
}

constexpr int RL_PROF_OFF = 200;

template <int GP, int Z, bool DAMP, bool COMBINE, bool PROF>
__global__ void __launch_bounds__(HW_MAX_THREADS, 3) fm_sgd_rowlane_kernel(const HogwildArgs a) {
  extern __shared__ __align__(128) unsigned char smem[];
  uint64_t* bars = reinterpret_cast<uint64_t*>(smem);
  float* s_acc = reinterpret_cast<float*>(smem + 64);
  unsigned long long* s_prof = reinterpret_cast<unsigned long long*>(smem + RL_PROF_OFF);

  const int tid = threadIdx.x;
  const int TR = a.tile_rows;
  const uint32_t G = gridDim.x;
  const uint32_t R = a.ramp_tiles;
  const uint32_t n_win = rowlane_windows(a.n_tiles, R, G);
  long long tprof = 0;
  auto prof_mark = [&](int slot) {
    if constexpr (PROF) {
      if (tid == 0) {
        const long long now = clock64();
        s_prof[slot] += (unsigned long long)(now - tprof);
        tprof = now;
      }
    }
  };
  if (PROF && tid < RL_PROF_SLOTS) s_prof[tid] = 0ull;
  auto tile_of = [&](uint32_t j) -> uint32_t {
    const uint32_t t = j < R ? (blockIdx.x == 0 ? j : HW_NO_TILE) : R + (j - R) * G + blockIdx.x;
    return t < a.n_tiles ? t : HW_NO_TILE;
  };

  const uint64_t policy = ring_init(smem, tid);
  const int ptid = (int)blockDim.x - 32;
  uint32_t pj = 0;
  auto next_tile = [&]() -> uint32_t {
    for (; pj < n_win; ++pj)
      if (tile_of(pj) != HW_NO_TILE) return tile_of(pj++);
    return HW_NO_TILE;
  };
  if (tid == ptid) {
    for (int i = 0; i < HW_NSTAGE; i++) {
      const uint32_t t = next_tile();
      if (t != HW_NO_TILE) {
        const uint64_t r0 = (uint64_t)t * TR, r1 = min(r0 + (uint64_t)TR, a.n_rows);
        issue_tile(a, smem, bars, t, i, policy, __ldg(a.row_ptr + r0), __ldg(a.row_ptr + r1));
      }
    }
  }
  __syncthreads();

  const bool use_w0 = a.use_w0 != 0;
  const float lr = a.lr;
  GridBarrier gbar{a.gbar, a.gbar_base};
  const uint64_t q0 = blockIdx.x * (uint64_t)blockDim.x + tid;
  const uint64_t fold_stride = (uint64_t)G * blockDim.x;
  const uint64_t n_vec = a.n_acc / 4;
  float4* state4 = reinterpret_cast<float4*>(a.state);
  ulonglong2* acc2 = reinterpret_cast<ulonglong2*>(a.acc);
  if (PROF && tid == 0) tprof = clock64();

  int it = 0;
  for (uint32_t j = 0; j < n_win; ++j) {
    const uint32_t tile = tile_of(j);
    if (tile != HW_NO_TILE) {
      const int stage = it % HW_NSTAGE;
      const uint32_t parity = (uint32_t)(it / HW_NSTAGE) & 1u;
      uint32_t nt = HW_NO_TILE;
      uint64_t nt_nb = 0, nt_ne = 0;
      if (tid == ptid) {
        nt = next_tile();
        if (nt != HW_NO_TILE) {
          const uint64_t r0 = (uint64_t)nt * TR, r1 = min(r0 + (uint64_t)TR, a.n_rows);
          nt_nb = __ldg(a.row_ptr + r0);
          nt_ne = __ldg(a.row_ptr + r1);
        }
      }
      HogwildArgs w = a;
      if (j < R) {
        w.conc_scale = a.ramp_conc_scale;
        w.w0_conc = a.ramp_w0_conc;
      }
      BiasFetch bias;
      bias.slot = reinterpret_cast<float*>(smem + 192);
      bias.issue(a, use_w0, tid);
      mbar_wait(bars + stage, parity);

      unsigned char* sb = stage_base(smem, a, stage);
      const uint64_t* rp = reinterpret_cast<const uint64_t*>(sb);
      const float* ys = reinterpret_cast<const float*>(sb + (size_t)(TR + 2) * 8);
      const uint32_t* ids = reinterpret_cast<const uint32_t*>(sb + (size_t)(TR + 2) * 8 + (size_t)TR * 4);
      const float* xs = reinterpret_cast<const float*>(ids + a.tile_cap);
      const uint64_t row0 = (uint64_t)tile * TR;
      const int rows_here = (int)min((uint64_t)TR, a.n_rows - row0);

      float mult, hj, w0 = 0.f;
      rowlane_tile<GP, Z, DAMP, COMBINE, true>(
          w, rp, ys, ids, xs, rows_here, tid,
          [&]() {
            w0 = bias.get(use_w0, tid, it, (int)blockDim.x);
            prof_mark(0);
            return w0;
          },
          mult, hj);
      float2* s_part = reinterpret_cast<float2*>(s_acc) + (it & 1) * 8;
      if (use_w0) bias_partial(s_part, mult, hj, tid);
      __syncthreads();
      if (tid == ptid) {
        if (nt != HW_NO_TILE) issue_tile(a, smem, bars, nt, stage, policy, nt_nb, nt_ne);
        if (use_w0) {
          float M = 0.f, H = 0.f;
          for (int i = 0; i < (int)(blockDim.x >> 5); i++) {
            M += s_part[i].x;
            H += s_part[i].y;
          }
          const float T = (float)rows_here;
          M += T * a.reg0 * w0;
          const float gsc = gamma_scale(fmaxf(w.w0_conc, 1.f), lr * (H / T + a.reg0));
          acc_add(a.acc_w0, -lr * gsc * M, a.acc_bad);
        }
      }
      ++it;
    }
    prof_mark(1);
    bulk_wait_all();
    fence_proxy_async_global();
    gbar.arrive(tid);
    prof_mark(2);
    float4 s = make_float4(0.f, 0.f, 0.f, 0.f);
    if (q0 < n_vec) s = __ldcg(state4 + q0);
    gbar.wait(tid);
    prof_mark(3);
    const bool bad = __ldcg(a.acc + a.n_acc) != 0ull;
    for (uint64_t q = q0; q < n_vec; q += fold_stride) {
      const ulonglong2 lo = __ldcg(acc2 + 2 * q), hi = __ldcg(acc2 + 2 * q + 1);
      if (q != q0) s = __ldcg(state4 + q);
      auto fold = [&](float& x, unsigned long long u) {
        if (bad) x = __int_as_float(0x7fffffff);
        else if (u != 0ull) x = x + (float)((double)(long long)u * (1.0 / (double)kAccScale));
      };
      fold(s.x, lo.x);
      fold(s.y, lo.y);
      fold(s.z, hi.x);
      fold(s.w, hi.y);
      if (bad || (lo.x | lo.y | hi.x | hi.y) != 0ull) state4[q] = s;
      if ((lo.x | lo.y) != 0ull) acc2[2 * q] = make_ulonglong2(0ull, 0ull);
      if ((hi.x | hi.y) != 0ull) acc2[2 * q + 1] = make_ulonglong2(0ull, 0ull);
    }
    prof_mark(4);
    if (j + 1 < n_win) {
      gbar.arrive(tid);
      gbar.wait(tid);
    }
    fence_proxy_async_global();
    prof_mark(5);
  }
  if constexpr (PROF) {
    __syncthreads();
    if (tid < RL_PROF_SLOTS) atomicAdd(a.prof + tid, s_prof[tid]);
  }
}


__device__ __forceinline__ void mbar_arrive(uint64_t* bar) {
  asm volatile("mbarrier.arrive.shared::cta.b64 _, [%0];" ::"r"(smem_u32(bar)) : "memory");
}

template <int GP, int Z, bool DAMP, bool COMBINE>
__global__ void __launch_bounds__(HW_MAX_THREADS + 32, 3) fm_sgd_rowlane_ws_kernel(const HogwildArgs a) {
  extern __shared__ __align__(128) unsigned char smem[];
  uint64_t* full = reinterpret_cast<uint64_t*>(smem);
  uint64_t* empty = reinterpret_cast<uint64_t*>(smem + 64);
  uint32_t* s_tile = reinterpret_cast<uint32_t*>(smem + 128);
  float* s_w0 = reinterpret_cast<float*>(smem + 160);
  float2* s_part = reinterpret_cast<float2*>(smem + 192);

  const int tid = threadIdx.x;
  const int lane = tid & 31;
  const int TR = a.tile_rows;
  const int n_cwarps = TR >> 5;
  const bool use_w0 = a.use_w0 != 0;
  auto stage_ptr = [&](int stage) { return smem + HW_WS_HDR_BYTES + (size_t)stage * a.stage_bytes; };

  if (tid == 0) {
    for (int i = 0; i < HW_NSTAGE; i++) {
      mbar_init(full + i, 1);
      mbar_init(empty + i, (uint32_t)n_cwarps);
    }
    fence_mbar_init();
  }
  __syncthreads();

  if (tid >= TR) {
    if (lane != 0) return;
    TileSched sched{a.sched, a.n_tiles, false};
    const uint64_t policy = policy_evict_first();
    auto fill = [&](int stage, uint32_t t) {
      s_tile[stage] = t;
      if (t == HW_NO_TILE) {
        mbar_arrive(full + stage);
        return;
      }
      s_w0[stage] = use_w0 ? ld_cg_f(a.w0) : 0.f;
      const uint64_t r0 = (uint64_t)t * TR, r1 = min(r0 + (uint64_t)TR, a.n_rows);
      issue_tile(a, smem, full, t, stage, policy, __ldg(a.row_ptr + r0), __ldg(a.row_ptr + r1), HW_WS_HDR_BYTES);
    };
    for (int i = 0; i < HW_NSTAGE; i++) fill(i, sched.claim());
    for (int it = 0;; ++it) {
      const int stage = it % HW_NSTAGE;
      const uint32_t t = s_tile[stage];
      if (t == HW_NO_TILE) break;
      mbar_wait(empty + stage, (uint32_t)(it / HW_NSTAGE) & 1u);
      if (use_w0) {
        float M = 0.f, H = 0.f;
        for (int i = 0; i < n_cwarps; i++) {
          const float2 p = s_part[stage * 8 + i];
          M += p.x;
          H += p.y;
        }
        const uint64_t row0 = (uint64_t)t * TR;
        const float T = (float)min((uint64_t)TR, a.n_rows - row0);
        M += T * a.reg0 * s_w0[stage];
        const float gsc = gamma_scale(fmaxf(a.w0_conc, 1.f), a.lr * (H / T + a.reg0));
        red_add_f(a.w0, -a.lr * gsc * M);
      }
      fill(stage, sched.claim());
    }
    sched.finish(gridDim.x, 0u);
    return;
  }

  for (int it = 0;; ++it) {
    const int stage = it % HW_NSTAGE;
    mbar_wait(full + stage, (uint32_t)(it / HW_NSTAGE) & 1u);
    const uint32_t tile = s_tile[stage];
    if (tile == HW_NO_TILE) break;
    unsigned char* sb = stage_ptr(stage);
    const uint64_t* rp = reinterpret_cast<const uint64_t*>(sb);
    const float* ys = reinterpret_cast<const float*>(sb + (size_t)(TR + 2) * 8);
    const uint32_t* ids = reinterpret_cast<const uint32_t*>(sb + (size_t)(TR + 2) * 8 + (size_t)TR * 4);
    const float* xs = reinterpret_cast<const float*>(ids + a.tile_cap);
    const uint64_t row0 = (uint64_t)tile * TR;
    const int rows_here = (int)min((uint64_t)TR, a.n_rows - row0);
    const float w0 = s_w0[stage];
    float mult, hj;
    rowlane_tile<GP, Z, DAMP, COMBINE, false>(a, rp, ys, ids, xs, rows_here, tid, [&]() { return w0; }, mult, hj);
    if (use_w0) bias_partial(s_part + stage * 8, mult, hj, tid);
    __syncwarp();
    if (lane == 0) mbar_arrive(empty + stage);
  }
}

template <int GP, int Z, bool PROF>
static HogwildKernelFn pick_d(bool damp, bool combine) {
  if (combine)
    return damp ? fm_sgd_rowlane_kernel<GP, Z, true, true, PROF> : fm_sgd_rowlane_kernel<GP, Z, false, true, PROF>;
  return damp ? fm_sgd_rowlane_kernel<GP, Z, true, false, PROF> : fm_sgd_rowlane_kernel<GP, Z, false, false, PROF>;
}

template <int GP, int Z>
static HogwildKernelFn pick_p(bool damp, bool combine, bool prof) {
  return prof ? pick_d<GP, Z, true>(damp, combine) : pick_d<GP, Z, false>(damp, combine);
}

template <int GP>
static HogwildKernelFn pick_z(int z, bool damp, bool combine, bool prof) {
  if (z <= 1) return pick_p<GP, 1>(damp, combine, prof);
  if (z <= 2) return pick_p<GP, 2>(damp, combine, prof);
  if (z <= 4) return pick_p<GP, 4>(damp, combine, prof);
  return nullptr;
}

template <int GP, int Z>
static HogwildKernelFn pick_d_ws(bool damp, bool combine) {
  if (combine)
    return damp ? fm_sgd_rowlane_ws_kernel<GP, Z, true, true> : fm_sgd_rowlane_ws_kernel<GP, Z, false, true>;
  return damp ? fm_sgd_rowlane_ws_kernel<GP, Z, true, false> : fm_sgd_rowlane_ws_kernel<GP, Z, false, false>;
}

template <int GP>
static HogwildKernelFn pick_z_ws(int z, bool damp, bool combine) {
  if (z <= 1) return pick_d_ws<GP, 1>(damp, combine);
  if (z <= 2) return pick_d_ws<GP, 2>(damp, combine);
  if (z <= 4) return pick_d_ws<GP, 4>(damp, combine);
  return nullptr;
}

HogwildKernelFn pick_rowlane_ws_kernel(int gp, int max_row_nnz, bool damp, bool combine) {
  if (gp == 1) return pick_z_ws<1>(max_row_nnz, damp, combine);
  if (gp == 2) return pick_z_ws<2>(max_row_nnz, damp, combine);
  return nullptr;
}

HogwildKernelFn pick_rowlane_kernel(int gp, int max_row_nnz, bool damp, bool combine, bool prof) {
  if (gp == 1) return pick_z<1>(max_row_nnz, damp, combine, prof);
  if (gp == 2) return pick_z<2>(max_row_nnz, damp, combine, prof);
  return nullptr;
}

}
```

libfm_b200/csrc/fmb200_internal.h:

```cpp
#pragma once
#include <cuda_runtime.h>
#include <stdint.h>

#include <memory>
#include <string>
#include <type_traits>

#include "../../include/fmb200.h"

namespace fmb {

struct CudaFree {
  void operator()(void* p) const { cudaFree(p); }
};
struct CudaFreeHost {
  void operator()(void* p) const { cudaFreeHost(p); }
};
struct CudaEventDestroy {
  void operator()(cudaEvent_t e) const { cudaEventDestroy(e); }
};
template <class T>
using DevPtr = std::unique_ptr<T, CudaFree>;
template <class T>
using HostPtr = std::unique_ptr<T, CudaFreeHost>;
using EventPtr = std::unique_ptr<std::remove_pointer_t<cudaEvent_t>, CudaEventDestroy>;

template <class T>
cudaError_t alloc(DevPtr<T>& p, uint64_t n) {
  p.reset();
  T* raw = nullptr;
  const cudaError_t e = cudaMalloc(&raw, (n ? n : 1) * sizeof(T));
  p.reset(raw);
  return e;
}

template <class T>
cudaError_t host_alloc(HostPtr<T>& p, size_t n) {
  p.reset();
  T* raw = nullptr;
  const cudaError_t e = cudaHostAlloc((void**)&raw, n * sizeof(T), cudaHostAllocDefault);
  p.reset(raw);
  return e;
}

inline cudaError_t event_create(EventPtr& p, unsigned int flags) {
  cudaEvent_t raw = nullptr;
  const cudaError_t e = cudaEventCreateWithFlags(&raw, flags);
  p.reset(raw);
  return e;
}

template <class T, class Cap>
cudaError_t grow(DevPtr<T>& p, Cap& cap, uint64_t n) {
  if (p && cap >= n) return cudaSuccess;
  cap = 0;
  const cudaError_t e = alloc(p, n);
  if (e == cudaSuccess) cap = (Cap)n;
  return e;
}

constexpr uint64_t kRowSlack = 512 + 8;
constexpr uint64_t kEntrySlack = 16;

struct DataSlot {
  bool present = false;
  uint64_t n_rows = 0;
  uint64_t nnz = 0;
  DevPtr<uint64_t> row_ptr;
  DevPtr<uint32_t> col;
  DevPtr<float> val;
  DevPtr<float> target;
  uint32_t max_row_nnz = 0;
  uint64_t cap_rows = 0, cap_nnz = 0;
  DevPtr<float> feat_cnt;
  DevPtr<unsigned int> d_flag;
  HostPtr<unsigned int> h_flag;
  EventPtr ready;
  bool pending = false;
  uint64_t upload_gen = 0;
  uint32_t max_feat_cnt = 0;
  uint32_t tile_span[5] = {0, 0, 0, 0, 0};
  DevPtr<uint32_t> link;
  DevPtr<uint32_t> rowdep;
  uint64_t link_cap = 0, rowdep_cap = 0;
  uint32_t* ord_shape = nullptr;
  bool links_ready = false;
  DevPtr<unsigned char> ord_scratch;
  size_t ord_scratch_bytes = 0;
};

constexpr int COMM_SEQ_WORD = 0;
constexpr int COMM_BAR_WORD = FMB200_MAX_PEERS;
constexpr int COMM_ROWS_WORD = 64;
constexpr int COMM_ROWS_PARITY_STRIDE = 16;
constexpr int COMM_MEAN_ROWS_WORD = 100;

constexpr int FMB_PEER_PART = 4096;

struct CommLayout {
  static constexpr size_t hdr_bytes = 1024;
  size_t buf_bytes = 0;
  size_t cnt_floats = 0;
  CommLayout() = default;
  CommLayout(uint64_t n_floats, uint32_t n_attr)
      : buf_bytes((n_floats * sizeof(float) + 255) & ~(size_t)255), cnt_floats(((size_t)n_attr + 63) & ~(size_t)63) {}
  size_t total_bytes() const { return hdr_bytes + 3 * buf_bytes + (3 * cnt_floats + 2 * (size_t)FMB_PEER_PART) * sizeof(float); }
  static unsigned int* words(unsigned char* b) { return reinterpret_cast<unsigned int*>(b); }
  unsigned int* rows_word(unsigned char* b, unsigned parity, int rank) const {
    return words(b) + COMM_ROWS_WORD + COMM_ROWS_PARITY_STRIDE * parity + rank;
  }
  float* buf(unsigned char* b, int i) const { return reinterpret_cast<float*>(b + hdr_bytes + (size_t)i * buf_bytes); }
  float* theta0(unsigned char* b) const { return buf(b, 2); }
  float* counts(unsigned char* b, unsigned parity) const {
    float* cnt0 = buf(b, 3);
    return parity ? cnt0 + 2 * cnt_floats + 2 * (size_t)FMB_PEER_PART : cnt0;
  }
  float* partials(unsigned char* b, int j) const { return counts(b, 0) + cnt_floats + (size_t)j * FMB_PEER_PART; }
  float* mean_counts(unsigned char* b) const { return partials(b, 2); }
};

struct Params32 {
  float* base = nullptr;
  uint64_t n_floats = 0;
  uint64_t off_w = 4;
  uint64_t off_v = 0;
  int ws = 1;
  __host__ __device__ float* w0() const { return base; }
  __host__ __device__ float* w() const { return base + off_w; }
  __host__ __device__ float* v() const { return base + off_v; }
};

struct Params64 {
  double* base = nullptr;
  uint64_t n_doubles = 0;
  uint64_t off_v = 0;
  static constexpr uint64_t off_w = 2;
  __host__ __device__ double* w0() const { return base; }
  __host__ __device__ double* w() const { return base + off_w; }
  __host__ __device__ double* v() const { return base + off_v; }
};

struct HParams {
  int task = 0;
  double lr = 0, reg0 = 0, regw = 0, regv = 0;
  double min_target = 0, max_target = 0;
};

struct McmcState;
struct McmcDelete {
  void operator()(McmcState* s) const;
};

struct EpochConfig {
  int lanes_per_row = 0, slots = 0, rows_per_tile = 0, grid = 0, block = 0, smem = 0, damp = 0;
};

}

struct fmb200_ctx {
  int device = 0;
  int sm_count = 0;
  int max_smem_optin = 0;
  cudaStream_t stream = nullptr;
  cudaStream_t copy_stream = nullptr;
  fmb::EventPtr ev0, ev1;
  uint32_t n = 0;
  int k = 0, kp = 0;
  bool k0 = true, k1 = true;
  int mode = FMB200_MODE_HOGWILD;
  fmb::HParams hp;
  fmb::Params32 p32;
  fmb::Params64 p64;
  fmb::DevPtr<double> p64_buf;
  fmb::DataSlot slots[FMB200_MAX_SLOTS];
  fmb::DevPtr<double> d_partials;
  uint64_t n_partials = 0;
  fmb::DevPtr<double> d_pred;
  uint64_t pred_cap = 0;
  fmb::DevPtr<unsigned int> d_sched;
  fmb::DevPtr<unsigned long long> d_acc;
  fmb::DevPtr<unsigned int> d_gbar;
  uint32_t gbar_count = 0;
  fmb::DevPtr<unsigned int> d_flag;
  fmb::HostPtr<unsigned int> h_flag;
  fmb::HostPtr<unsigned char> h_stage;
  uint64_t launches = 0;
  fmb::EpochConfig last_cfg;
  int tune_ctas_per_sm = 0, tune_rows_per_tile = 0, tune_threads = 0;
  fmb::DevPtr<unsigned char> comm_base;
  fmb::CommLayout comm;
  bool peer_base_valid = false;
  bool hogwild_fresh = true;
  int peer_part_cur = 0, peer_n_part = 0;
  unsigned char* peer_base[FMB200_MAX_PEERS] = {nullptr};
  bool peer_ipc[FMB200_MAX_PEERS] = {false};
  int peer_world = 1, peer_rank = 0, peer_cur = 0;
  unsigned int peer_seq = 0, peer_bar_seq = 0;
  uint64_t peer_cnt_stamp[2] = {0, 0};
  uint64_t upload_counter = 0;
  fmb::DevPtr<double> sgda_grad_w, sgda_grad_v, sgda_reg_w, sgda_reg_v;
  fmb::DevPtr<uint32_t> sgda_group;
  uint32_t sgda_groups = 0;
  int tune_damp = 0;
  int tune_variant = 0;
  std::unique_ptr<fmb::McmcState, fmb::McmcDelete> mcmc;
};

namespace fmb {

inline int grid_for(const fmb200_ctx* c, uint64_t work) {
  const uint64_t blocks = (work + 255) / 256, cap = (uint64_t)c->sm_count * 8;
  return (int)(blocks < 1 ? 1 : (blocks < cap ? blocks : cap));
}

cudaError_t launch_sgd_inorder(fmb200_ctx* c, const DataSlot& d);
cudaError_t launch_predict64(fmb200_ctx* c, const DataSlot& d, int transform, double* out_pred,
                             double* partials, int n_blocks);
cudaError_t launch_sgd_ordered(fmb200_ctx* c, DataSlot& d, bool* handled);
struct SortedEntries {
  const uint32_t* ids = nullptr;
  const uint32_t* ent = nullptr;
};
cudaError_t build_ordered_links(fmb200_ctx* c, DataSlot& d, SortedEntries* sorted = nullptr);
cudaError_t launch_mcmc_eterms(fmb200_ctx* c, const DataSlot& d, double* e_out);
std::string mcmc_begin(fmb200_ctx* c, int train, int test, int do_sample, int do_multilevel, uint32_t n_groups,
                       const uint32_t* attr_group, const uint32_t* attr_per_group, double reg0,
                       const double* w_lambda0, const double* v_lambda0);
std::string mcmc_iteration(fmb200_ctx* c, double* train_metric, uint32_t* counters);
bool mcmc_get(const fmb200_ctx* c, double* alpha, double* w_mu, double* w_lambda, double* v_mu, double* v_lambda,
              double* pred_this, double* pred_sum_all, double* pred_sum_all_but5, uint32_t* n_runs);
cudaError_t launch_sgda_epoch(fmb200_ctx* c, const DataSlot& tr, const DataSlot& va, int lambda_steps);
cudaError_t launch_sgd_hogwild(fmb200_ctx* c, const DataSlot& d);
cudaError_t clear_acc_flag(fmb200_ctx* c);
cudaError_t launch_predict32(fmb200_ctx* c, const DataSlot& d, int transform, double* out_pred,
                             double* partials, int n_blocks);
cudaError_t launch_p64_to_p32(fmb200_ctx* c);
cudaError_t launch_p32_to_p64(fmb200_ctx* c);
cudaError_t launch_scale_p32(fmb200_ctx* c, float factor);
cudaError_t launch_peer_mean(fmb200_ctx* c);
cudaError_t launch_peer_barrier(fmb200_ctx* c);
cudaError_t peer_preload_kernels();
cudaError_t launch_peer_meanfield(fmb200_ctx* c);
cudaError_t peer_before_epoch(fmb200_ctx* c, const DataSlot& d);
cudaError_t launch_csr_inspect(fmb200_ctx* c, cudaStream_t st, const uint64_t* rp, uint64_t n_rows, uint64_t nnz,
                               unsigned int* out8);
cudaError_t launch_feature_counts(fmb200_ctx* c, cudaStream_t st, const uint32_t* col, uint64_t nnz, float* cnt,
                                  unsigned int* out_max_id, unsigned int* out_max);

cudaError_t launch_aos_to_csr(fmb200_ctx* c, cudaStream_t st, const void* d_rows, const void* d_entries, uint64_t n_rows,
                              uint64_t nnz, unsigned long long host_base_ptr, unsigned long long* scratch,
                              uint64_t* row_ptr, uint32_t* col, float* val, unsigned int* flag);
cudaError_t launch_aos_split(fmb200_ctx* c, cudaStream_t st, const void* d_entries, uint64_t nnz, uint32_t* col, float* val);
uint64_t aos_scan_tiles(uint64_t n_rows);
cudaError_t launch_onehot_fill(fmb200_ctx* c, cudaStream_t st, uint64_t n_rows, uint32_t z, uint64_t* row_ptr, float* val);

void pick_geometry(int kp, uint64_t n_rows, uint64_t nnz, int* G, int* S, int* cls);

}
```

libfm_b200/model.py:

```python
from __future__ import annotations

import ctypes as C
import math

import numpy as np

from . import _capi

TASK_REGRESSION = 0
TASK_CLASSIFICATION = 1
MODE_INORDER = 0
MODE_HOGWILD = 1
MODE_ORDERED = 2


class FmError(RuntimeError):
    """The reference throws std::string / const char* (caught at libfm.cpp:436-440)."""


def _p(arr, typ):
    return arr.ctypes.data_as(C.POINTER(typ))


class Data:

    def __init__(self, row_ptr, col, val, target, num_feature=None):
        self.row_ptr = np.ascontiguousarray(row_ptr, dtype=np.uint64)
        self.col = np.ascontiguousarray(col, dtype=np.uint32)
        self.val = np.ascontiguousarray(val, dtype=np.float32)
        self.target = np.ascontiguousarray(target, dtype=np.float32)
        self.num_cases = int(self.row_ptr.shape[0] - 1)
        if num_feature is None:
            num_feature = int(self.col.max()) + 1 if self.col.size else 0
        self.num_feature = int(num_feature)
        if self.target.size:
            self.min_target = float(self.target.min())
            self.max_target = float(self.target.max())
        else:
            self.min_target = float(np.finfo(np.float32).max)
            self.max_target = -float(np.finfo(np.float32).max)

    @property
    def num_values(self) -> int:
        return int(self.row_ptr[-1])

    def rows(self, lo, hi) -> "Data":
        a, b = int(self.row_ptr[lo]), int(self.row_ptr[hi])
        return Data(self.row_ptr[lo:hi + 1] - self.row_ptr[lo], self.col[a:b], self.val[a:b],
                    self.target[lo:hi], self.num_feature)

    def binarize_targets(self) -> None:
        self.target = np.where(self.target <= 0.0, -1.0, 1.0).astype(np.float32)

    @staticmethod
    def load(filename: str) -> "Data":
        row_ptr = [0]
        col, val, target = [], [], []
        try:
            f = open(filename, "r")
        except OSError:
            raise FmError("unable to open " + filename)
        with f:
            for line in f:
                s = line.strip(" \t\r\n")
                if not s or s[0] == "#":
                    continue
                tok = s.split()
                try:
                    target.append(np.float32(tok[0]))
                    for t in tok[1:]:
                        if t[0] == "#":
                            break
                        i, v = t.split(":")
                        col.append(int(i))
                        val.append(np.float32(v))
                except (ValueError, IndexError):
                    raise FmError('cannot parse line "' + line.rstrip("\n") + '"')
                row_ptr.append(len(col))
        return Data(np.array(row_ptr, dtype=np.uint64), np.array(col, dtype=np.uint32),
                    np.array(val, dtype=np.float32), np.array(target, dtype=np.float32))


def pinned_copy(arr: np.ndarray) -> np.ndarray:
    lib = _capi.load()
    p = C.c_void_p()
    if lib.fmb200_host_alloc(C.byref(p), arr.nbytes) != 0:
        raise FmError(lib.fmb200_last_error().decode())
    buf = (C.c_char * max(arr.nbytes, 1)).from_address(p.value)
    out = np.frombuffer(buf, dtype=arr.dtype, count=arr.size).reshape(arr.shape)
    out[...] = arr
    return out


class _LibcRand:

    def __init__(self):
        self.libc = C.CDLL(None)
        self.libc.rand.restype = C.c_int
        self.libc.srand.argtypes = [C.c_uint]

    def srand(self, seed: int) -> None:
        self.libc.srand(C.c_uint(seed & 0xFFFFFFFF))

    def uniform(self) -> float:
        return self.libc.rand() / (2147483647.0 + 1.0)

    def gaussian(self) -> float:
        while True:
            u = self.uniform()
            while u == 0.0:
                u = self.uniform()
            v = 1.7156 * (self.uniform() - 0.5)
            x = u - 0.449871
            y = abs(v) + 0.386595
            q = x * x + y * (0.19600 * y - 0.25472 * x)
            if q < 0.27597:
                break
            if not ((q > 0.27846) or ((v * v) > (-4.0 * u * u * math.log(u)))):
                break
        return v / u


class FmModel:

    def __init__(self, num_attribute: int, num_factor: int, k0: bool = True, k1: bool = True):
        self.num_attribute = int(num_attribute)
        self.num_factor = int(num_factor)
        self.k0, self.k1 = bool(k0), bool(k1)
        self.reg0 = self.regw = self.regv = 0.0
        self.init_mean = 0.0
        self.init_stdev = 0.01
        self.w0 = 0.0
        self.w = np.zeros(self.num_attribute, dtype=np.float64)
        self.v = np.zeros((self.num_factor, self.num_attribute), dtype=np.float64)

    def init(self, seed: int | None = None) -> None:
        rng = _LibcRand()
        if seed is not None:
            rng.srand(seed)
        self.w0 = 0.0
        self.w[:] = 0.0
        if self.init_stdev == 0.0 or math.isnan(self.init_stdev):
            self.v[:] = self.init_mean
            return
        flat = self.v.reshape(-1)
        for i in range(flat.shape[0]):
            flat[i] = self.init_mean + self.init_stdev * rng.gaussian()

    def init_numpy(self, seed: int) -> None:
        r = np.random.default_rng(seed)
        self.w0 = 0.0
        self.w[:] = 0.0
        self.v[:] = self.init_mean + self.init_stdev * r.standard_normal(self.v.shape)

    def saveModel(self, path: str) -> None:
        def g(x):
            return "%g" % x
        with open(path, "w") as f:
            if self.k0:
                f.write("#global bias W0\n" + g(self.w0) + "\n")
            if self.k1:
                f.write("#unary interactions Wj\n")
                for i in range(self.num_attribute):
                    f.write(g(self.w[i]) + "\n")
            f.write("#pairwise interactions Vj,f\n")
            for i in range(self.num_attribute):
                f.write(" ".join(g(self.v[q, i]) for q in range(self.num_factor)) + "\n")


class FmLearnSgdElement:

    def __init__(self, fm: FmModel, device: int = 0, mode: int = MODE_HOGWILD):
        self.lib = _capi.load()
        self.fm = fm
        self.task = TASK_REGRESSION
        self.learn_rate = 0.0
        self.num_iter = 100
        self.min_target = 0.0
        self.max_target = 0.0
        self.mode = mode
        self._ctx = C.c_void_p()
        self._check(self.lib.fmb200_create(C.byref(self._ctx), device, fm.num_attribute,
                                           fm.num_factor, int(fm.k0), int(fm.k1)))
        self._check(self.lib.fmb200_set_mode(self._ctx, mode))
        self._slots = {}
        self.push_params()

    def _check(self, rc: int) -> None:
        if rc != 0:
            raise FmError(self.lib.fmb200_last_error().decode())

    def close(self) -> None:
        if self._ctx:
            self.lib.fmb200_destroy(self._ctx)
            self._ctx = C.c_void_p()

    def __del__(self):
        try:
            self.close()
        except Exception:
            pass

    def set_mode(self, mode: int) -> None:
        self._check(self.lib.fmb200_set_mode(self._ctx, mode))
        self.mode = mode

    def set_tuning(self, ctas_per_sm=0, rows_per_tile=0, threads=0, damp=0, variant=0) -> None:
        self._check(self.lib.fmb200_set_tuning(self._ctx, ctas_per_sm, rows_per_tile, threads, damp,
                                               variant))

    def push_hparams(self) -> None:
        self._check(self.lib.fmb200_set_hparams(self._ctx, self.task, self.learn_rate, self.fm.reg0,
                                                self.fm.regw, self.fm.regv, self.min_target,
                                                self.max_target))

    def push_params(self) -> None:
        fm = self.fm
        w = np.ascontiguousarray(fm.w, dtype=np.float64)
        v = np.ascontiguousarray(fm.v, dtype=np.float64)
        self._check(self.lib.fmb200_set_params(self._ctx, float(fm.w0), _p(w, C.c_double),
                                               _p(v, C.c_double)))

    def pull_params(self) -> None:
        fm = self.fm
        w0 = C.c_double()
        w = np.empty(fm.num_attribute, dtype=np.float64)
        v = np.empty((fm.num_factor, fm.num_attribute), dtype=np.float64)
        self._check(self.lib.fmb200_get_params(self._ctx, C.byref(w0), _p(w, C.c_double),
                                               _p(v, C.c_double)))
        fm.w0, fm.w, fm.v = w0.value, w, v

    def upload(self, data: Data, slot: int) -> None:
        self._check(self.lib.fmb200_upload_data(
            self._ctx, slot, data.num_cases, data.num_values, _p(data.row_ptr, C.c_uint64),
            _p(data.col, C.c_uint32), _p(data.val, C.c_float), _p(data.target, C.c_float)))
        for key in [k for k, (s, _) in self._slots.items() if s == slot]:
            del self._slots[key]
        self._slots[id(data)] = (slot, data)

    def upload_onehot(self, data: Data, slot: int) -> None:
        z = data.num_values // max(data.num_cases, 1)
        if data.num_values != z * data.num_cases or not np.all(data.val == 1.0) or \
                not np.array_equal(data.row_ptr, np.arange(data.num_cases + 1, dtype=np.uint64) * np.uint64(z)):
            raise FmError("upload_onehot needs fixed-width rows with every value 1")
        self._check(self.lib.fmb200_upload_onehot(self._ctx, slot, data.num_cases, z,
                                                  _p(data.col, C.c_uint32), _p(data.target, C.c_float)))
        for key in [k for k, (s, _) in self._slots.items() if s == slot]:
            del self._slots[key]
        self._slots[id(data)] = (slot, data)

    def upload_aos(self, data: Data, slot: int, contiguous: bool = True) -> None:
        ent = np.empty(max(data.num_values, 1), dtype=[("id", np.uint32), ("value", np.float32)])
        ent["id"][:data.num_values] = data.col
        ent["value"][:data.num_values] = data.val
        rows = np.zeros(max(data.num_cases, 1), dtype=[("data", np.uint64), ("size", np.uint32), ("pad", np.uint32)])
        sizes = np.diff(data.row_ptr.astype(np.int64)).astype(np.uint32)
        keep = [ent]
        if contiguous:
            rows["data"][:data.num_cases] = ent.ctypes.data + 8 * data.row_ptr[:-1]
        else:
            for r in range(data.num_cases):
                a, b = int(data.row_ptr[r]), int(data.row_ptr[r + 1])
                part = ent[a:b].copy()
                keep.append(part)
                rows["data"][r] = part.ctypes.data
        rows["size"][:data.num_cases] = sizes
        self._check(self.lib.fmb200_upload_data_aos(self._ctx, slot, data.num_cases,
                                                    rows.ctypes.data_as(C.c_void_p), _p(data.target, C.c_float)))
        del keep
        for key in [k for k, (s, _) in self._slots.items() if s == slot]:
            del self._slots[key]
        self._slots[id(data)] = (slot, data)

    def release(self, data: Data) -> None:
        ent = self._slots.pop(id(data), None)
        if ent is not None:
            self._check(self.lib.fmb200_free_data(self._ctx, ent[0]))

    def _slot_of(self, data: Data) -> int:
        if id(data) not in self._slots:
            used = {s for s, _ in self._slots.values()}
            free = [s for s in range(8) if s not in used]
            if not free:
                raise FmError("all 8 data slots are in use: release() one first")
            self.upload(data, free[0])
        return self._slots[id(data)][0]

    def sgd_epoch(self, train: Data) -> float:
        sec = C.c_double()
        self._check(self.lib.fmb200_sgd_epoch(self._ctx, self._slot_of(train), C.byref(sec)))
        return sec.value

    def evaluate(self, data: Data) -> float:
        sq, ab, ok = C.c_double(), C.c_double(), C.c_uint64()
        self._check(self.lib.fmb200_evaluate(self._ctx, self._slot_of(data), C.byref(sq),
                                             C.byref(ab), C.byref(ok)))
        self.last_mae = ab.value / max(1, data.num_cases)
        if self.task == TASK_REGRESSION:
            return math.sqrt(sq.value / data.num_cases)
        return ok.value / data.num_cases

    def predict(self, data: Data, transform: bool = True) -> np.ndarray:
        out = np.empty(data.num_cases, dtype=np.float64)
        self._check(self.lib.fmb200_predict(self._ctx, self._slot_of(data), int(transform),
                                            _p(out, C.c_double)))
        return out

    def sgda_begin(self, attr_group=None) -> None:
        if attr_group is None:
            self._sgda_groups = 1
            self._check(self.lib.fmb200_sgda_begin(self._ctx, 1, None))
        else:
            g = np.ascontiguousarray(attr_group, dtype=np.uint32)
            self._sgda_groups = int(g.max()) + 1
            self._check(self.lib.fmb200_sgda_begin(self._ctx, self._sgda_groups, _p(g, C.c_uint32)))

    def sgda_epoch(self, train: Data, validation: Data, lambda_steps: bool) -> float:
        sec = C.c_double()
        self._check(self.lib.fmb200_sgda_epoch(self._ctx, self._slot_of(train), self._slot_of(validation),
                                               int(lambda_steps), C.byref(sec)))
        return sec.value

    def sgda_reg(self):
        reg_w = np.zeros(self._sgda_groups)
        reg_v = np.zeros((self._sgda_groups, self.fm.num_factor))
        self._check(self.lib.fmb200_sgda_get_reg(self._ctx, _p(reg_w, C.c_double), _p(reg_v, C.c_double)))
        return reg_w, reg_v

    def mcmc_eterms(self, data: Data) -> np.ndarray:
        out = np.empty(data.num_cases, dtype=np.float64)
        self._check(self.lib.fmb200_mcmc_eterms(self._ctx, self._slot_of(data), _p(out, C.c_double)))
        return out

    def mcmc_begin(self, train: Data, test: Data, do_sample: bool, do_multilevel: bool, reg0: float,
                   w_lambda, v_lambda, attr_group=None, attr_per_group=None) -> None:
        self.push_hparams()
        wl = np.ascontiguousarray(w_lambda, dtype=np.float64)
        self._mcmc_groups = int(wl.shape[0])
        vl = np.ascontiguousarray(v_lambda, dtype=np.float64).reshape(self._mcmc_groups, self.fm.num_factor)
        g = None if attr_group is None else np.ascontiguousarray(attr_group, dtype=np.uint32)
        pg = None if attr_per_group is None else np.ascontiguousarray(attr_per_group, dtype=np.uint32)
        self._check(self.lib.fmb200_mcmc_begin(
            self._ctx, self._slot_of(train), self._slot_of(test), int(do_sample), int(do_multilevel),
            self._mcmc_groups, None if g is None else _p(g, C.c_uint32), None if pg is None else _p(pg, C.c_uint32),
            float(reg0), _p(wl, C.c_double), _p(vl, C.c_double)))

    def mcmc_iteration(self):
        m = C.c_double()
        cnt = np.zeros(16, dtype=np.uint32)
        self._check(self.lib.fmb200_mcmc_iteration(self._ctx, C.byref(m), _p(cnt, C.c_uint32)))
        return m.value, cnt

    def mcmc_hyper(self) -> dict:
        G, k = self._mcmc_groups, self.fm.num_factor
        alpha = C.c_double()
        out = {"w_mu": np.zeros(G), "w_lambda": np.zeros(G), "v_mu": np.zeros((G, k)), "v_lambda": np.zeros((G, k))}
        self._check(self.lib.fmb200_mcmc_get_hyper(self._ctx, C.byref(alpha), *[_p(out[n], C.c_double) for n in
                                                                               ("w_mu", "w_lambda", "v_mu", "v_lambda")]))
        out["alpha"] = alpha.value
        return out

    def mcmc_pred(self, test: Data):
        out = [np.zeros(test.num_cases) for _ in range(3)]
        self._check(self.lib.fmb200_mcmc_get_pred(self._ctx, *[_p(a, C.c_double) for a in out]))
        return tuple(out)

    def mcmc_runs(self) -> int:
        n = C.c_uint32()
        self._check(self.lib.fmb200_mcmc_runs(self._ctx, C.byref(n)))
        return n.value

    def learn(self, train: Data, test: Data, log=None):
        self.push_hparams()
        hist = []
        for i in range(self.num_iter):
            t = self.sgd_epoch(train)
            tr, te = self.evaluate(train), self.evaluate(test)
            hist.append((tr, te, t))
            if log is not None:
                log("#Iter=%3d\tTrain=%g\tTest=%g" % (i, tr, te))
        self.pull_params()
        return hist

    def params_device(self):
        ptr, n = C.c_void_p(), C.c_uint64()
        self._check(self.lib.fmb200_params_device(self._ctx, C.byref(ptr), C.byref(n)))
        return ptr.value, n.value

    def params_layout(self) -> dict:
        off_w, off_v, ws, kp = C.c_uint64(), C.c_uint64(), C.c_int(), C.c_int()
        self._check(self.lib.fmb200_params_layout(self._ctx, C.byref(off_w), C.byref(ws), C.byref(off_v), C.byref(kp)))
        return {"off_w": off_w.value, "ws": ws.value, "off_v": off_v.value, "kp": kp.value,
                "n": self.fm.num_attribute}

    def stream(self) -> int:
        s = C.c_void_p()
        self._check(self.lib.fmb200_stream(self._ctx, C.byref(s)))
        return s.value or 0

    def kernel_launches(self) -> int:
        n = C.c_uint64()
        self._check(self.lib.fmb200_kernel_launches(self._ctx, C.byref(n)))
        return n.value

    def download(self, slot: int) -> Data:
        nr, nz = C.c_uint64(), C.c_uint64()
        self._check(self.lib.fmb200_download_data(self._ctx, slot, C.byref(nr), C.byref(nz), None, None, None, None))
        rp = np.zeros(nr.value + 1, dtype=np.uint64)
        col = np.zeros(max(nz.value, 1), dtype=np.uint32)
        val = np.zeros(max(nz.value, 1), dtype=np.float32)
        tg = np.zeros(max(nr.value, 1), dtype=np.float32)
        self._check(self.lib.fmb200_download_data(self._ctx, slot, None, None, _p(rp, C.c_uint64),
                                                  _p(col, C.c_uint32), _p(val, C.c_float), _p(tg, C.c_float)))
        return Data(rp, col[:nz.value], val[:nz.value], tg[:nr.value], 0)

    def ordered_index(self, data: Data):
        link = np.empty(max(data.num_values, 1), dtype=np.uint32)
        rowdep = np.empty(max(data.num_cases, 1), dtype=np.uint32)
        self._check(self.lib.fmb200_ordered_index(self._ctx, self._slot_of(data), _p(link, C.c_uint32),
                                                  _p(rowdep, C.c_uint32)))
        return link[:data.num_values], rowdep[:data.num_cases]

    def epoch_config(self) -> dict:
        v = [C.c_int() for _ in range(7)]
        self._check(self.lib.fmb200_last_epoch_config(self._ctx, *[C.byref(x) for x in v]))
        keys = ["lanes_per_row", "slots", "rows_per_tile", "grid", "block", "smem_bytes", "damp"]
        return dict(zip(keys, [x.value for x in v]))
```

Baseline: 5.967 billion.

## Deal hogwild rows into per-window sorted CSR copy with deferred bias accumulation

Adds a precomputed dealt copy of the training CSR, made at upload time by radix-sorting rows within each grid window by their last column id. This is meant to improve locality and reduce conflicts in the hogwild rowlane kernel. A new kernel variant reads the permuted arrays. It moves the w0 bias reduction to a per-row buffer that is folded at the window barrier through a double-buffered accumulator. The cost is extra device memory, a sort at upload, an extra global barrier per window, and more complex NaN and bias handling.

```diff
diff --git a/include/fmb200.h b/include/fmb200.h
--- a/include/fmb200.h
+++ b/include/fmb200.h
@@ -91,6 +91,7 @@
 int fmb200_kernel_launches(fmb200_ctx* ctx, uint64_t* count);
 int fmb200_last_epoch_config(fmb200_ctx* ctx, int* lanes_per_row, int* slots, int* rows_per_tile,
                              int* grid, int* block, int* smem_bytes, int* damp);
+int fmb200_last_epoch_dealt(fmb200_ctx* ctx, int* dealt);
 int fmb200_set_tuning(fmb200_ctx* ctx, int ctas_per_sm, int rows_per_tile, int threads, int damp,
                       int variant);
 int fmb200_ordered_index(fmb200_ctx* ctx, int slot, uint32_t* link ,
diff --git a/libfm_b200/_capi.py b/libfm_b200/_capi.py
--- a/libfm_b200/_capi.py
+++ b/libfm_b200/_capi.py
@@ -57,6 +57,7 @@
     "fmb200_download_data": (C.c_int, [_ctx, C.c_int, _u64p, _u64p, _u64p, _u32p, _f32p, _f32p]),
     "fmb200_kernel_launches": (C.c_int, [_ctx, _u64p]),
     "fmb200_last_epoch_config": (C.c_int, [_ctx] + [_intp] * 7),
+    "fmb200_last_epoch_dealt": (C.c_int, [_ctx, _intp]),
     "fmb200_set_tuning": (C.c_int, [_ctx, C.c_int, C.c_int, C.c_int, C.c_int, C.c_int]),
     "fmb200_ordered_index": (C.c_int, [_ctx, C.c_int, _u32p, _u32p]),
 }
diff --git a/libfm_b200/build.py b/libfm_b200/build.py
--- a/libfm_b200/build.py
+++ b/libfm_b200/build.py
@@ -28,6 +28,7 @@
     "fm_inorder.cu": ["--fmad=false"],
     "fm_ordered.cu": [],
     "fm_upload.cu": [],
+    "fm_deal.cu": [],
     "fm_mcmc.cu": ["--fmad=false"],
 }
 CU_HEADERS = ["fm_device.cuh", "fm_rowgroup.cuh", "fm_hogwild_common.cuh", "fmb200_internal.h",
diff --git a/libfm_b200/csrc/fm_context.cu b/libfm_b200/csrc/fm_context.cu
--- a/libfm_b200/csrc/fm_context.cu
+++ b/libfm_b200/csrc/fm_context.cu
@@ -75,6 +75,7 @@
   s.present = false;
   s.links_ready = false;
   s.upload_gen = ++c->upload_counter;
+  s.hogwild_epochs = 0;
   s.n_rows = n_rows;
   s.nnz = nnz;
   return 0;
@@ -114,7 +115,7 @@
   return upload_inspect(c, slot, st);
 }
 
-int upload_finish(fmb200_ctx* c, int slot) {
+int upload_finish(fmb200_ctx* c, int slot, bool deal = false) {
   DataSlot& s = c->slots[slot];
   if (!s.pending) return 0;
   CK(cudaEventSynchronize(s.ready.get()));
@@ -130,13 +131,14 @@
   for (int i = 0; i < 5; i++) s.tile_span[i] = h[2 + i];
   s.max_feat_cnt = h[9];
   s.present = true;
+  if (deal) CK(prepare_rowlane_deal(c, s));
   return 0;
 }
 
 int upload_common(fmb200_ctx* c, int slot, uint64_t n_rows, uint64_t nnz, const uint64_t* row_ptr,
                   const uint32_t* col, const float* val, const float* target) {
   if (upload_enqueue(c, slot, n_rows, nnz, row_ptr, col, val, target, c->stream)) return 1;
-  return upload_finish(c, slot);
+  return upload_finish(c, slot, true);
 }
 
 int need_slot(fmb200_ctx* c, int slot) {
@@ -388,7 +390,7 @@
   CK(cudaMemcpyAsync(s.target.get(), target, n_rows * sizeof(float), cudaMemcpyHostToDevice, st));
   CK(launch_aos_split(c, st, d_ent.get(), nnz, s.col.get(), s.val.get()));
   if (upload_inspect(c, slot, st)) return 1;
-  return upload_finish(c, slot);
+  return upload_finish(c, slot, true);
 }
 
 int fmb200_upload_onehot(fmb200_ctx* c, int slot, uint64_t n_rows, uint32_t nnz_per_row,
@@ -399,7 +401,7 @@
   if (n_rows > 0xffffffffull) return fail("row count exceeds the reference's uint range");
   if (bind(c)) return 1;
   if (upload_onehot_enqueue(c, slot, n_rows, nnz_per_row, ids, target, c->stream)) return 1;
-  return upload_finish(c, slot);
+  return upload_finish(c, slot, true);
 }
 
 int fmb200_upload_onehot_async(fmb200_ctx* c, int slot, uint64_t n_rows, uint32_t nnz_per_row,
@@ -879,6 +881,12 @@
   return 0;
 }
 
+int fmb200_last_epoch_dealt(fmb200_ctx* c, int* dealt) {
+  NEED_CTX(c);
+  if (dealt) *dealt = c->last_cfg.dealt;
+  return 0;
+}
+
 int fmb200_download_data(fmb200_ctx* c, int slot, uint64_t* n_rows, uint64_t* nnz, uint64_t* row_ptr,
                          uint32_t* col, float* val, float* target) {
   NEED_CTX(c);
diff --git a/libfm_b200/csrc/fm_deal.cu b/libfm_b200/csrc/fm_deal.cu
--- /dev/null
+++ b/libfm_b200/csrc/fm_deal.cu
@@ -0,0 +1,110 @@
+#include <cub/device/device_radix_sort.cuh>
+#include <cub/device/device_scan.cuh>
+
+#include "fmb200_internal.h"
+
+namespace fmb {
+
+namespace {
+
+__global__ void deal_key_kernel(const uint64_t* __restrict__ rp, const uint32_t* __restrict__ col, uint64_t n_rows,
+                                uint64_t win_rows, uint32_t n, uint64_t* __restrict__ key, uint32_t* __restrict__ row) {
+  for (uint64_t r = blockIdx.x * (uint64_t)blockDim.x + threadIdx.x; r < n_rows; r += (uint64_t)gridDim.x * blockDim.x) {
+    const uint64_t b = rp[r], e = rp[r + 1];
+    key[r] = (r / win_rows) * ((uint64_t)n + 1) + (e > b ? col[e - 1] : n);
+    row[r] = (uint32_t)r;
+  }
+}
+
+__global__ void deal_rows_kernel(const uint64_t* __restrict__ rp, const float* __restrict__ tgt,
+                                 const uint32_t* __restrict__ perm, uint64_t n_rows, uint64_t win_rows,
+                                 uint64_t* __restrict__ len, float* __restrict__ dtgt, uint32_t* __restrict__ pos) {
+  for (uint64_t i = blockIdx.x * (uint64_t)blockDim.x + threadIdx.x; i <= n_rows; i += (uint64_t)gridDim.x * blockDim.x) {
+    if (i == n_rows) {
+      len[i] = 0;
+      continue;
+    }
+    const uint32_t r = perm[i];
+    len[i] = rp[r + 1] - rp[r];
+    dtgt[i] = tgt[r];
+    pos[i] = (uint32_t)(r % win_rows);
+  }
+}
+
+__global__ void deal_entries_kernel(const uint64_t* __restrict__ rp, const uint32_t* __restrict__ col,
+                                    const float* __restrict__ val, const uint32_t* __restrict__ perm, uint64_t n_rows,
+                                    const uint64_t* __restrict__ drp, uint32_t* __restrict__ dcol,
+                                    float* __restrict__ dval) {
+  for (uint64_t i = blockIdx.x * (uint64_t)blockDim.x + threadIdx.x; i < n_rows; i += (uint64_t)gridDim.x * blockDim.x) {
+    const uint32_t r = perm[i];
+    const uint64_t b = rp[r], n = rp[r + 1] - b, o = drp[i];
+    for (uint64_t k = 0; k < n; k++) {
+      dcol[o + k] = col[b + k];
+      dval[o + k] = val[b + k];
+    }
+  }
+}
+
+}
+
+cudaError_t build_rowlane_deal(fmb200_ctx* c, DataSlot& d, int TR, uint32_t G) {
+  RowlaneDeal& dl = d.deal;
+  if (dl.matches(d.upload_gen, TR, G)) return cudaSuccess;
+  if (d.n_rows >= 0xffffffffull) return cudaErrorInvalidValue;
+  const uint64_t n_rows = d.n_rows, win_rows = (uint64_t)G * TR;
+  const uint64_t n_win = (n_rows + win_rows - 1) / win_rows;
+  int bits = 1;
+  while (bits < 64 && ((n_win * ((uint64_t)c->n + 1)) >> bits) != 0) bits++;
+  cudaError_t e;
+  const uint64_t cap_r = d.cap_rows + kRowSlack, cap_e = d.cap_nnz + kEntrySlack;
+  if (dl.rows_cap < cap_r || dl.nnz_cap < cap_e) {
+    if ((e = alloc(dl.row_ptr, cap_r + 1)) != cudaSuccess) return e;
+    if ((e = alloc(dl.target, cap_r)) != cudaSuccess) return e;
+    if ((e = alloc(dl.pos, cap_r)) != cudaSuccess) return e;
+    if ((e = alloc(dl.col, cap_e)) != cudaSuccess) return e;
+    if ((e = alloc(dl.val, cap_e)) != cudaSuccess) return e;
+    if ((e = cudaMemsetAsync(dl.row_ptr.get(), 0, (cap_r + 1) * sizeof(uint64_t), c->stream)) != cudaSuccess) return e;
+    if ((e = cudaMemsetAsync(dl.target.get(), 0, cap_r * sizeof(float), c->stream)) != cudaSuccess) return e;
+    if ((e = cudaMemsetAsync(dl.col.get(), 0, cap_e * sizeof(uint32_t), c->stream)) != cudaSuccess) return e;
+    if ((e = cudaMemsetAsync(dl.val.get(), 0, cap_e * sizeof(float), c->stream)) != cudaSuccess) return e;
+    dl.rows_cap = cap_r;
+    dl.nnz_cap = cap_e;
+  }
+  size_t sort_bytes = 0, scan_bytes = 0;
+  if ((e = cub::DeviceRadixSort::SortPairs(nullptr, sort_bytes, (const uint64_t*)nullptr, (uint64_t*)nullptr,
+                                           (const uint32_t*)nullptr, (uint32_t*)nullptr, n_rows, 0, bits,
+                                           c->stream)) != cudaSuccess)
+    return e;
+  if ((e = cub::DeviceScan::ExclusiveSum(nullptr, scan_bytes, (const uint64_t*)nullptr, (uint64_t*)nullptr,
+                                         n_rows + 1, c->stream)) != cudaSuccess)
+    return e;
+  const size_t words = (n_rows + 1 + 63) & ~(uint64_t)63;
+  const size_t need = 3 * words * 8 + 2 * words * 4 + std::max(sort_bytes, scan_bytes) + 256;
+  if ((e = grow(dl.scratch, dl.scratch_bytes, need)) != cudaSuccess) return e;
+  uint64_t* key_in = reinterpret_cast<uint64_t*>(dl.scratch.get());
+  uint64_t* key_out = key_in + words;
+  uint64_t* len = key_out + words;
+  uint32_t* row_in = reinterpret_cast<uint32_t*>(len + words);
+  uint32_t* perm = row_in + words;
+  void* tmp = perm + words;
+  const int grid = grid_for(c, n_rows + 1);
+  deal_key_kernel<<<grid, 256, 0, c->stream>>>(d.row_ptr.get(), d.col.get(), n_rows, win_rows, c->n, key_in, row_in);
+  if ((e = cub::DeviceRadixSort::SortPairs(tmp, sort_bytes, key_in, key_out, row_in, perm, n_rows, 0, bits,
+                                           c->stream)) != cudaSuccess)
+    return e;
+  deal_rows_kernel<<<grid, 256, 0, c->stream>>>(d.row_ptr.get(), d.target.get(), perm, n_rows, win_rows, len,
+                                                dl.target.get(), dl.pos.get());
+  if ((e = cub::DeviceScan::ExclusiveSum(tmp, scan_bytes, len, dl.row_ptr.get(), n_rows + 1, c->stream)) !=
+      cudaSuccess)
+    return e;
+  deal_entries_kernel<<<grid, 256, 0, c->stream>>>(d.row_ptr.get(), d.col.get(), d.val.get(), perm, n_rows,
+                                                   dl.row_ptr.get(), dl.col.get(), dl.val.get());
+  if ((e = cudaGetLastError()) != cudaSuccess) return e;
+  c->launches += 5;
+  dl.gen = d.upload_gen;
+  dl.tr = TR;
+  dl.grid = G;
+  return cudaSuccess;
+}
+
+}
diff --git a/libfm_b200/csrc/fm_hogwild.cu b/libfm_b200/csrc/fm_hogwild.cu
--- a/libfm_b200/csrc/fm_hogwild.cu
+++ b/libfm_b200/csrc/fm_hogwild.cu
@@ -317,6 +317,9 @@
   a.gbar = nullptr;
   a.gbar_base = 0;
   a.prof = nullptr;
+  a.deal_pos = nullptr;
+  a.bias_rows = nullptr;
+  a.acc_w0x = nullptr;
   a.sched = c->d_sched.get();
   a.global_entries = 0;
   return a;
@@ -328,36 +331,79 @@
   return c->d_acc ? cudaMemsetAsync(acc_flag(c), 0, sizeof(unsigned long long), c->stream) : cudaSuccess;
 }
 
-static cudaError_t launch_rowlane(fmb200_ctx* c, const DataSlot& d, bool* handled) {
-  *handled = false;
+struct RowlanePlan {
+  int threads = 0, TR = 0, launch_threads = 0, grid = 0;
+  uint32_t cap = 0, sbytes = 0, cap_dealt = 0, sbytes_dealt = 0;
+  int smem = 0, smem_dealt = 0;
+  bool damp = false, combine = false, ws = false, prof = false, dealable = false;
+  HogwildKernelFn fn = nullptr, fn_dealt = nullptr;
+};
+
+static cudaError_t plan_rowlane(fmb200_ctx* c, const DataSlot& d, RowlanePlan* p, bool* ok) {
+  *ok = false;
   const int gp = c->kp / 4;
-  if (gp < 1 || gp > 2 || d.max_row_nnz > 4 || c->tune_variant == 1) return cudaSuccess;
+  if (gp < 1 || gp > 2 || d.max_row_nnz > 4 || c->tune_variant == 1 || d.n_rows == 0) return cudaSuccess;
   int threads = c->tune_threads > 0 ? std::min(c->tune_threads, HW_MAX_THREADS) : 256;
   int tr_idx = 0;
   while ((32 << (tr_idx + 1)) <= threads) tr_idx++;
-  threads = 32 << tr_idx;
-  const int TR = threads;
-  const uint32_t cap = (d.tile_span[tr_idx] + 3u) & ~3u;
-  const uint32_t sbytes = (uint32_t)hw_stage_bytes(TR, cap);
-  const bool damp = want_damp(c, d, 3.0 * TR);
-  const bool combine = (double)d.max_feat_cnt * 32.0 / (double)d.n_rows > 0.5;
-  const bool ws = c->tune_variant == 3;
-  const bool want_prof = c->tune_variant == 132;
-  HogwildKernelFn fn = ws ? pick_rowlane_ws_kernel(gp, (int)d.max_row_nnz, damp, combine)
-                          : pick_rowlane_kernel(gp, (int)d.max_row_nnz, damp, combine, want_prof);
-  if (fn == nullptr) return cudaSuccess;
-  const int smem = (ws ? HW_WS_HDR_BYTES : HW_HDR_BYTES) + HW_NSTAGE * (int)sbytes;
-  const int launch_threads = ws ? threads + 32 : threads;
+  p->threads = 32 << tr_idx;
+  p->TR = p->threads;
+  p->cap = (d.tile_span[tr_idx] + 3u) & ~3u;
+  p->sbytes = (uint32_t)hw_stage_bytes(p->TR, p->cap);
+  p->damp = want_damp(c, d, 3.0 * p->TR);
+  p->combine = (double)d.max_feat_cnt * 32.0 / (double)d.n_rows > 0.5;
+  p->ws = c->tune_variant == 3;
+  p->prof = c->tune_variant == 132 || c->tune_variant == 133;
+  p->fn = p->ws ? pick_rowlane_ws_kernel(gp, (int)d.max_row_nnz, p->damp, p->combine)
+                : pick_rowlane_kernel(gp, (int)d.max_row_nnz, p->damp, p->combine, p->prof, false);
+  if (p->fn == nullptr) return cudaSuccess;
+  p->smem = (p->ws ? HW_WS_HDR_BYTES : HW_HDR_BYTES) + HW_NSTAGE * (int)p->sbytes;
+  p->launch_threads = p->ws ? p->threads + 32 : p->threads;
+  const uint64_t n_tiles = (d.n_rows + p->TR - 1) / p->TR;
+  cudaError_t e = fit_grid(c, p->fn, p->launch_threads, p->smem, n_tiles, &p->grid);
+  if (e != cudaSuccess) return e;
+  *ok = true;
+  if (p->ws || p->combine || c->tune_variant == 5 || c->tune_variant == 133) return cudaSuccess;
+  p->fn_dealt = pick_rowlane_kernel(gp, (int)d.max_row_nnz, p->damp, false, p->prof, true);
+  p->cap_dealt = std::max<uint32_t>(p->cap, (uint32_t)p->TR * d.max_row_nnz + 4u);
+  p->sbytes_dealt = (uint32_t)hw_stage_bytes(p->TR, p->cap_dealt);
+  p->smem_dealt = HW_HDR_BYTES + HW_NSTAGE * (int)p->sbytes_dealt;
+  int grid_dealt = 0;
+  if ((e = fit_grid(c, p->fn_dealt, p->threads, p->smem_dealt, n_tiles, &grid_dealt)) != cudaSuccess) return e;
+  p->dealable = grid_dealt == p->grid;
+  return cudaSuccess;
+}
+
+cudaError_t prepare_rowlane_deal(fmb200_ctx* c, DataSlot& d) {
+  if (c->mode != FMB200_MODE_HOGWILD || c->kp == 0) return cudaSuccess;
+  RowlanePlan p;
+  bool ok = false;
+  cudaError_t e = plan_rowlane(c, d, &p, &ok);
+  if (e != cudaSuccess || !ok || !p.dealable) return e;
+  return build_rowlane_deal(c, d, p.TR, (uint32_t)p.grid);
+}
+
+static cudaError_t launch_rowlane(fmb200_ctx* c, DataSlot& d, bool* handled) {
+  *handled = false;
+  RowlanePlan p;
+  bool ok = false;
+  cudaError_t e = plan_rowlane(c, d, &p, &ok);
+  if (e != cudaSuccess || !ok) return e;
+  const int TR = p.TR;
+  const int grid = p.grid;
   const uint64_t n_tiles = (d.n_rows + TR - 1) / TR;
-  int grid = 0;
-  cudaError_t e = fit_grid(c, fn, launch_threads, smem, n_tiles, &grid);
-  if (e != cudaSuccess) return e;
-  HogwildArgs a = make_args(c, d, n_tiles, TR, cap, sbytes);
-  a.conc_scale = (float)(std::min<double>((double)d.n_rows, (double)grid * TR) / (double)d.n_rows);
-  a.w0_conc = (float)std::min<double>((double)d.n_rows, (double)grid * TR * (ws ? HW_NSTAGE : 1));
+  const bool ws = p.ws, want_prof = p.prof;
   constexpr uint64_t kRampTiles = 4;
   const bool ramp = c->hogwild_fresh && c->k0 && c->tune_damp >= 0 && n_tiles > 8 * kRampTiles;
   c->hogwild_fresh = false;
+  const bool dealt = p.dealable && !ramp && (d.deal.matches(d.upload_gen, TR, (uint32_t)grid) || d.hogwild_epochs > 0);
+  d.hogwild_epochs++;
+  HogwildKernelFn fn = dealt ? p.fn_dealt : p.fn;
+  const int smem = dealt ? p.smem_dealt : p.smem;
+  const int launch_threads = p.launch_threads;
+  HogwildArgs a = make_args(c, d, n_tiles, TR, dealt ? p.cap_dealt : p.cap, dealt ? p.sbytes_dealt : p.sbytes);
+  a.conc_scale = (float)(std::min<double>((double)d.n_rows, (double)grid * TR) / (double)d.n_rows);
+  a.w0_conc = (float)std::min<double>((double)d.n_rows, (double)grid * TR * (ws ? HW_NSTAGE : 1));
   if (ws) {
     if (ramp) {
       HogwildArgs r = a;
@@ -397,6 +443,22 @@
       a.ramp_conc_scale = (float)((double)TR / (double)d.n_rows);
       a.ramp_w0_conc = (float)TR;
     }
+    if (dealt) {
+      if ((e = build_rowlane_deal(c, d, TR, (uint32_t)grid)) != cudaSuccess) return e;
+      a.row_ptr = d.deal.row_ptr.get();
+      a.col = d.deal.col.get();
+      a.val = d.deal.val.get();
+      a.target = d.deal.target.get();
+      a.deal_pos = d.deal.pos.get();
+      const uint64_t words = 2 + (uint64_t)grid * TR;
+      if (c->deal_bias_cap < words) {
+        if ((e = grow(c->d_deal_bias, c->deal_bias_cap, words)) != cudaSuccess) return e;
+        if ((e = cudaMemsetAsync(c->d_deal_bias.get(), 0, 2 * sizeof(unsigned long long), c->stream)) != cudaSuccess)
+          return e;
+      }
+      a.acc_w0x = c->d_deal_bias.get();
+      a.bias_rows = reinterpret_cast<float2*>(c->d_deal_bias.get() + 2);
+    }
     a.gbar = c->d_gbar.get();
     a.gbar_base = c->gbar_count;
     if (want_prof) {
@@ -413,7 +475,7 @@
     }
     c->launches++;
     const uint32_t n_win = rowlane_windows(a.n_tiles, a.ramp_tiles, (uint32_t)grid);
-    c->gbar_count += (uint32_t)grid * rowlane_barriers(a.n_tiles, a.ramp_tiles, (uint32_t)grid);
+    c->gbar_count += (uint32_t)grid * rowlane_barriers(a.n_tiles, a.ramp_tiles, (uint32_t)grid, dealt);
     if (want_prof) {
       unsigned long long h[RL_PROF_SLOTS];
       if ((e = cudaMemcpyAsync(h, a.prof, sizeof(h), cudaMemcpyDeviceToHost, c->stream)) != cudaSuccess) return e;
@@ -426,12 +488,13 @@
       fprintf(stderr, "\n");
     }
   }
-  c->last_cfg = EpochConfig{1, (int)std::max<uint32_t>(1, d.max_row_nnz), TR, grid, launch_threads, smem, damp ? 1 : 0};
+  c->last_cfg = EpochConfig{1, (int)std::max<uint32_t>(1, d.max_row_nnz), TR, grid, launch_threads, smem,
+                            p.damp ? 1 : 0, dealt ? 1 : 0};
   *handled = true;
   return cudaGetLastError();
 }
 
-cudaError_t launch_sgd_hogwild(fmb200_ctx* c, const DataSlot& d) {
+cudaError_t launch_sgd_hogwild(fmb200_ctx* c, DataSlot& d) {
   if (c->kp / 4 > 32) return cudaErrorInvalidValue;
   if (d.n_rows == 0) return cudaSuccess;
   {
diff --git a/libfm_b200/csrc/fm_hogwild_common.cuh b/libfm_b200/csrc/fm_hogwild_common.cuh
--- a/libfm_b200/csrc/fm_hogwild_common.cuh
+++ b/libfm_b200/csrc/fm_hogwild_common.cuh
@@ -50,13 +50,16 @@
   unsigned int* gbar;
   uint32_t gbar_base;
   unsigned long long* prof;
+  const uint32_t* deal_pos;
+  float2* bias_rows;
+  unsigned long long* acc_w0x;
 };
 
 __host__ __device__ inline uint32_t rowlane_windows(uint32_t n_tiles, uint32_t ramp, uint32_t G) {
   return ramp + (n_tiles - ramp + G - 1) / G;
 }
-__host__ __device__ inline uint32_t rowlane_barriers(uint32_t n_tiles, uint32_t ramp, uint32_t G) {
-  return 2u * rowlane_windows(n_tiles, ramp, G) - 1u;
+__host__ __device__ inline uint32_t rowlane_barriers(uint32_t n_tiles, uint32_t ramp, uint32_t G, bool dealt) {
+  return 2u * rowlane_windows(n_tiles, ramp, G) - (dealt ? 0u : 1u);
 }
 
 struct GridBarrier {
@@ -86,6 +89,11 @@
   if (fabsf(d) < kAccStepMax) return (unsigned long long)__float2ll_rn(d * kAccScale);
   atomicOr(bad, 1ull);
   return 0ull;
+}
+
+__device__ __forceinline__ float acc_fold(float x, unsigned long long u, bool bad) {
+  if (bad) return __int_as_float(0x7fffffff);
+  return u != 0ull ? x + (float)((double)(long long)u * (1.0 / (double)kAccScale)) : x;
 }
 
 __device__ __forceinline__ unsigned char* stage_base(unsigned char* smem, const HogwildArgs& a,
@@ -215,7 +223,7 @@
 
 using HogwildKernelFn = void (*)(const HogwildArgs);
 
-HogwildKernelFn pick_rowlane_kernel(int gp, int max_row_nnz, bool damp, bool combine, bool prof);
+HogwildKernelFn pick_rowlane_kernel(int gp, int max_row_nnz, bool damp, bool combine, bool prof, bool dealt);
 constexpr int RL_PROF_SLOTS = 6;
 HogwildKernelFn pick_rowlane_ws_kernel(int gp, int max_row_nnz, bool damp, bool combine);
 
diff --git a/libfm_b200/csrc/fm_rowlane.cu b/libfm_b200/csrc/fm_rowlane.cu
--- a/libfm_b200/csrc/fm_rowlane.cu
+++ b/libfm_b200/csrc/fm_rowlane.cu
@@ -9,24 +9,58 @@
   float v[4 * GP];
 };
 
+template <int GP>
+__device__ __forceinline__ unsigned long long* wb_slot(int e, int tid) {
+  __shared__ __align__(128) unsigned long long s_wb[2][HW_MAX_THREADS][4 * GP];
+  return s_wb[e & 1][tid];
+}
+template <int GP, int Z, typename Q>
+__device__ __forceinline__ void acc_add_row_q(unsigned long long* acc_v, uint32_t id, bool live, int e, int tid, Q q) {
+  constexpr int K = 4 * GP;
+  unsigned long long* slot = wb_slot<GP>(e, tid);
+  bulk_wait_read<Z == 1 ? 0 : 1>();
+  if (live) {
+#pragma unroll
+    for (int f = 0; f < K; f += 2) *reinterpret_cast<ulonglong2*>(slot + f) = make_ulonglong2(q(f), q(f + 1));
+    fence_proxy_async_shared();
+    bulk_red_add_u64(acc_v + (size_t)id * K, slot, K * 8);
+  }
+  bulk_commit();
+}
 template <int GP, int Z>
 __device__ __forceinline__ void acc_add_row(unsigned long long* acc_v, uint32_t id, bool live,
                                             const float (&d)[4 * GP], int e, int tid, unsigned long long* bad) {
-  constexpr int K = 4 * GP;
-  __shared__ __align__(128) unsigned long long s_wb[2][HW_MAX_THREADS][K];
-  unsigned long long* slot = s_wb[e & 1][tid];
-  bulk_wait_read<Z == 1 ? 0 : 1>();
-  if (live) {
-#pragma unroll
-    for (int f = 0; f < K; f += 2)
-      *reinterpret_cast<ulonglong2*>(slot + f) = make_ulonglong2(acc_quantise(d[f], bad), acc_quantise(d[f + 1], bad));
-    fence_proxy_async_shared();
-    bulk_red_add_u64(acc_v + (size_t)id * K, slot, K * 8);
-  }
-  bulk_commit();
-}
-
-template <int GP, int Z, bool DAMP, bool COMBINE, bool ACC, typename W0F>
+  acc_add_row_q<GP, Z>(acc_v, id, live, e, tid, [&](int f) { return acc_quantise(d[f], bad); });
+}
+
+template <int GP>
+__device__ __forceinline__ FactorRow<GP> gather_row(const float4* V4, uint32_t gid, int odd) {
+  FactorRow<GP> r;
+  const float4 zero4 = make_float4(0.f, 0.f, 0.f, 0.f);
+  if constexpr (GP == 2) {
+    const uint32_t pid = __shfl_xor_sync(0xffffffffu, gid, 1);
+    const uint32_t idA = odd ? pid : gid;
+    const uint32_t idB = odd ? gid : pid;
+    const float4 la = idA != 0xffffffffu ? ld_cg_f4(V4 + (size_t)idA * 2 + odd) : zero4;
+    const float4 lb = idB != 0xffffffffu ? ld_cg_f4(V4 + (size_t)idB * 2 + odd) : zero4;
+    const float4 send = odd ? la : lb;
+    float4 recv;
+    recv.x = __shfl_xor_sync(0xffffffffu, send.x, 1);
+    recv.y = __shfl_xor_sync(0xffffffffu, send.y, 1);
+    recv.z = __shfl_xor_sync(0xffffffffu, send.z, 1);
+    recv.w = __shfl_xor_sync(0xffffffffu, send.w, 1);
+    const float4 lo = odd ? recv : la;
+    const float4 hi = odd ? lb : recv;
+    r.v[0] = lo.x; r.v[1] = lo.y; r.v[2] = lo.z; r.v[3] = lo.w;
+    r.v[4] = hi.x; r.v[5] = hi.y; r.v[6] = hi.z; r.v[7] = hi.w;
+  } else {
+    const float4 l = gid != 0xffffffffu ? ld_cg_f4(V4 + (size_t)gid) : zero4;
+    r.v[0] = l.x; r.v[1] = l.y; r.v[2] = l.z; r.v[3] = l.w;
+  }
+  return r;
+}
+
+template <int GP, int Z, bool DAMP, bool COMBINE, bool ACC, bool DEALT, typename W0F>
 __device__ __forceinline__ void rowlane_tile(const HogwildArgs& a, const uint64_t* rp,
                                              const float* ys, const uint32_t* ids,
                                              const float* xs, int rows_here, int tid, W0F get_w0,
@@ -56,31 +90,36 @@
     id[e] = on ? ids[beg + e] : 0u;
     x[e] = on ? xs[beg + e] : 0.f;
   }
+  const int kq = DEALT ? cnt - 1 : -1;
+  uint32_t kid = 0xffffffffu;
+#pragma unroll
+  for (int e = 0; e < Z; ++e)
+    if (e == kq) kid = id[e];
+  int seg = lane;
+  if (DEALT) {
+    const uint32_t prev = __shfl_up_sync(0xffffffffu, kid, 1);
+    const bool head = lane == 0 || kid == 0xffffffffu || prev != kid;
+    seg = 31 - __clz(__ballot_sync(0xffffffffu, head) & (0xffffffffu >> (31 - lane)));
+  }
 #pragma unroll
   for (int e = 0; e < Z; ++e) {
-    if (GP == 2) {
-      const uint32_t gid = (e < cnt) ? id[e] : 0xffffffffu;
-      const uint32_t pid = __shfl_xor_sync(0xffffffffu, gid, 1);
-      const uint32_t idA = odd ? pid : gid;
-      const uint32_t idB = odd ? gid : pid;
-      const float4 zero4 = make_float4(0.f, 0.f, 0.f, 0.f);
-      const float4 la = idA != 0xffffffffu ? ld_cg_f4(V4 + (size_t)idA * 2 + odd) : zero4;
-      const float4 lb = idB != 0xffffffffu ? ld_cg_f4(V4 + (size_t)idB * 2 + odd) : zero4;
-      const float4 send = odd ? la : lb;
-      float4 recv;
-      recv.x = __shfl_xor_sync(0xffffffffu, send.x, 1);
-      recv.y = __shfl_xor_sync(0xffffffffu, send.y, 1);
-      recv.z = __shfl_xor_sync(0xffffffffu, send.z, 1);
-      recv.w = __shfl_xor_sync(0xffffffffu, send.w, 1);
-      const float4 lo = odd ? recv : la;
-      const float4 hi = odd ? lb : recv;
-      vr[e].v[0] = lo.x; vr[e].v[1] = lo.y; vr[e].v[2] = lo.z; vr[e].v[3] = lo.w;
-      vr[e].v[4] = hi.x; vr[e].v[5] = hi.y; vr[e].v[6] = hi.z; vr[e].v[7] = hi.w;
-    } else {
-      const float4 l = (e < cnt) ? ld_cg_f4(V4 + (size_t)id[e]) : make_float4(0.f, 0.f, 0.f, 0.f);
-      vr[e].v[0] = l.x; vr[e].v[1] = l.y; vr[e].v[2] = l.z; vr[e].v[3] = l.w;
-    }
-    wv[e] = (use_w && e < cnt) ? ld_cg_f(a.w + (size_t)id[e] * a.ws) : 0.f;
+    const bool fetch = e < cnt && e != kq;
+    vr[e] = gather_row<GP>(V4, fetch ? id[e] : 0xffffffffu, odd);
+    wv[e] = (use_w && fetch) ? ld_cg_f(a.w + (size_t)id[e] * a.ws) : 0.f;
+  }
+  if (DEALT) {
+    const bool fetch = lane == seg && kid != 0xffffffffu;
+    FactorRow<GP> kv = gather_row<GP>(V4, fetch ? kid : 0xffffffffu, odd);
+    float kw = (use_w && fetch) ? ld_cg_f(a.w + (size_t)kid * a.ws) : 0.f;
+#pragma unroll
+    for (int f = 0; f < K; ++f) kv.v[f] = __shfl_sync(0xffffffffu, kv.v[f], seg);
+    kw = __shfl_sync(0xffffffffu, kw, seg);
+#pragma unroll
+    for (int e = 0; e < Z; ++e)
+      if (e == kq) {
+        vr[e] = kv;
+        wv[e] = kw;
+      }
   }
 
   float sum[K];
@@ -113,6 +152,16 @@
   const float hrow = (use_w ? xx : 0.f) + fmaxf((xx - 2.f) * s2 + sq, 0.f);
   const float hjoint = DAMP ? curv * ((use_w0 ? 1.f : 0.f) + hrow) : curv;
 
+  struct KeyStep {
+    float v[K], w;
+  } kd{};
+  auto make_kd = [](const float (&d)[K], float dw) {
+    KeyStep k;
+#pragma unroll
+    for (int f = 0; f < K; ++f) k.v[f] = d[f];
+    k.w = dw;
+    return k;
+  };
   const float nlr_mult = -lr * mult;
   const float nlr_regv = -lr * a.regv;
   const float nlr_regw = -lr * a.regw;
@@ -134,6 +183,10 @@
       d[f] = sv * (nlr_mult * (sum[f] * x[e] - vr[e].v[f] * x2) + nlr_regv * vr[e].v[f]);
     float dw = sw * (nlr_mult * x[e] + nlr_regw * wv[e]);
     bool on_c = on;
+    if (DEALT && e == kq) {
+      kd = make_kd(d, dw);
+      on_c = false;
+    }
     if (COMBINE) {
       const uint32_t key = on ? id[e] : (0x80000000u | (uint32_t)lane);
       unsigned peers = __match_any_sync(0xffffffffu, key);
@@ -192,6 +245,25 @@
       else red_add_f(a.w + (size_t)id[e] * a.ws, dw);
     }
   }
+  if constexpr (DEALT) {
+    const bool has_key = kid != 0xffffffffu;
+    unsigned long long q[K + 1];
+#pragma unroll
+    for (int f = 0; f < K; ++f) q[f] = has_key ? acc_quantise(kd.v[f], a.acc_bad) : 0ull;
+    q[K] = (has_key && use_w) ? acc_quantise(kd.w, a.acc_bad) : 0ull;
+#pragma unroll
+    for (int s = 1; s < 32; s <<= 1) {
+      const bool take = __shfl_down_sync(0xffffffffu, seg, s) == seg && lane + s < 32;
+#pragma unroll
+      for (int f = 0; f <= K; ++f) {
+        const unsigned long long t = __shfl_down_sync(0xffffffffu, q[f], s);
+        if (take) q[f] += t;
+      }
+    }
+    const bool issue = has_key && lane == seg;
+    acc_add_row_q<GP, Z>(a.acc_v, kid, issue, Z, tid, [&](int f) { return q[f]; });
+    if (issue && use_w) red_add_u64(a.acc_w + (size_t)kid * a.ws, q[K]);
+  }
 
   mult_out = mult;
   hjoint_out = valid ? hjoint : 0.f;
@@ -199,7 +271,7 @@
 
 constexpr int RL_PROF_OFF = 200;
 
-template <int GP, int Z, bool DAMP, bool COMBINE, bool PROF>
+template <int GP, int Z, bool DAMP, bool COMBINE, bool PROF, bool DEALT>
 __global__ void __launch_bounds__(HW_MAX_THREADS, 3) fm_sgd_rowlane_kernel(const HogwildArgs a) {
   extern __shared__ __align__(128) unsigned char smem[];
   uint64_t* bars = reinterpret_cast<uint64_t*>(smem);
@@ -256,9 +328,12 @@
   ulonglong2* acc2 = reinterpret_cast<ulonglong2*>(a.acc);
   if (PROF && tid == 0) tprof = clock64();
 
+  float w0_run = (DEALT && use_w0 && tid == 0) ? ld_cg_f(a.w0) : 0.f;
+  bool bad = false;
   int it = 0;
   for (uint32_t j = 0; j < n_win; ++j) {
     const uint32_t tile = tile_of(j);
+    if (DEALT && use_w0 && tid == 0 && j > 0) w0_run = acc_fold(w0_run, __ldcg(a.acc_w0x + ((j - 1) & 1)), bad);
     if (tile != HW_NO_TILE) {
       const int stage = it % HW_NSTAGE;
       const uint32_t parity = (uint32_t)(it / HW_NSTAGE) & 1u;
@@ -279,7 +354,11 @@
       }
       BiasFetch bias;
       bias.slot = reinterpret_cast<float*>(smem + 192);
-      bias.issue(a, use_w0, tid);
+      if (DEALT) bias.pending = w0_run;
+      else bias.issue(a, use_w0, tid);
+      const uint32_t pos = DEALT && tid < (int)min((uint64_t)TR, a.n_rows - (uint64_t)tile * TR)
+                               ? __ldg(a.deal_pos + (uint64_t)tile * TR + tid)
+                               : 0xffffffffu;
       mbar_wait(bars + stage, parity);
 
       unsigned char* sb = stage_base(smem, a, stage);
@@ -291,7 +370,7 @@
       const int rows_here = (int)min((uint64_t)TR, a.n_rows - row0);
 
       float mult, hj, w0 = 0.f;
-      rowlane_tile<GP, Z, DAMP, COMBINE, true>(
+      rowlane_tile<GP, Z, DAMP, COMBINE, true, DEALT>(
           w, rp, ys, ids, xs, rows_here, tid,
           [&]() {
             w0 = bias.get(use_w0, tid, it, (int)blockDim.x);
@@ -300,11 +379,15 @@
           },
           mult, hj);
       float2* s_part = reinterpret_cast<float2*>(s_acc) + (it & 1) * 8;
-      if (use_w0) bias_partial(s_part, mult, hj, tid);
+      if (DEALT) {
+        if (use_w0 && pos != 0xffffffffu) a.bias_rows[pos] = make_float2(mult, hj);
+      } else if (use_w0) {
+        bias_partial(s_part, mult, hj, tid);
+      }
       __syncthreads();
       if (tid == ptid) {
         if (nt != HW_NO_TILE) issue_tile(a, smem, bars, nt, stage, policy, nt_nb, nt_ne);
-        if (use_w0) {
+        if (!DEALT && use_w0) {
           float M = 0.f, H = 0.f;
           for (int i = 0; i < (int)(blockDim.x >> 5); i++) {
             M += s_part[i].x;
@@ -327,29 +410,56 @@
     if (q0 < n_vec) s = __ldcg(state4 + q0);
     gbar.wait(tid);
     prof_mark(3);
-    const bool bad = __ldcg(a.acc + a.n_acc) != 0ull;
+    float2 pr = make_float2(0.f, 0.f);
+    if (DEALT && use_w0 && tile != HW_NO_TILE && tid < (int)min((uint64_t)TR, a.n_rows - (uint64_t)tile * TR))
+      pr = __ldcg(a.bias_rows + blockIdx.x * TR + tid);
+    bad = __ldcg(a.acc + a.n_acc) != 0ull;
     for (uint64_t q = q0; q < n_vec; q += fold_stride) {
       const ulonglong2 lo = __ldcg(acc2 + 2 * q), hi = __ldcg(acc2 + 2 * q + 1);
       if (q != q0) s = __ldcg(state4 + q);
-      auto fold = [&](float& x, unsigned long long u) {
-        if (bad) x = __int_as_float(0x7fffffff);
-        else if (u != 0ull) x = x + (float)((double)(long long)u * (1.0 / (double)kAccScale));
-      };
-      fold(s.x, lo.x);
-      fold(s.y, lo.y);
-      fold(s.z, hi.x);
-      fold(s.w, hi.y);
+      s.x = acc_fold(s.x, lo.x, bad);
+      s.y = acc_fold(s.y, lo.y, bad);
+      s.z = acc_fold(s.z, hi.x, bad);
+      s.w = acc_fold(s.w, hi.y, bad);
       if (bad || (lo.x | lo.y | hi.x | hi.y) != 0ull) state4[q] = s;
       if ((lo.x | lo.y) != 0ull) acc2[2 * q] = make_ulonglong2(0ull, 0ull);
       if ((hi.x | hi.y) != 0ull) acc2[2 * q + 1] = make_ulonglong2(0ull, 0ull);
     }
+    if (DEALT && use_w0) {
+      if (tile != HW_NO_TILE) {
+        float2* s_part = reinterpret_cast<float2*>(s_acc);
+        bias_partial(s_part, pr.x, pr.y, tid);
+        __syncthreads();
+        if (tid == 0) {
+          float M = 0.f, H = 0.f;
+          for (int i = 0; i < (int)(blockDim.x >> 5); i++) {
+            M += s_part[i].x;
+            H += s_part[i].y;
+          }
+          const float T = (float)min((uint64_t)TR, a.n_rows - (uint64_t)tile * TR);
+          M += T * a.reg0 * w0_run;
+          const float gsc = gamma_scale(fmaxf(a.w0_conc, 1.f), lr * (H / T + a.reg0));
+          acc_add(a.acc_w0x + (j & 1), -lr * gsc * M, a.acc_bad);
+        }
+      }
+      if (blockIdx.x == 0 && tid == 0 && j > 0) a.acc_w0x[(j - 1) & 1] = 0ull;
+    }
     prof_mark(4);
-    if (j + 1 < n_win) {
+    if (DEALT || j + 1 < n_win) {
       gbar.arrive(tid);
       gbar.wait(tid);
     }
     fence_proxy_async_global();
     prof_mark(5);
+  }
+  if (DEALT) {
+    const bool bad_end = __ldcg(a.acc + a.n_acc) != 0ull;
+    if (bad_end && !bad)
+      for (uint64_t q = q0; q < n_vec; q += fold_stride) state4[q] = make_float4(NAN, NAN, NAN, NAN);
+    if (use_w0 && blockIdx.x == 0 && tid == 0) {
+      *a.w0 = acc_fold(w0_run, __ldcg(a.acc_w0x + ((n_win - 1) & 1)), bad_end);
+      a.acc_w0x[(n_win - 1) & 1] = 0ull;
+    }
   }
   if constexpr (PROF) {
     __syncthreads();
@@ -440,7 +550,8 @@
     const int rows_here = (int)min((uint64_t)TR, a.n_rows - row0);
     const float w0 = s_w0[stage];
     float mult, hj;
-    rowlane_tile<GP, Z, DAMP, COMBINE, false>(a, rp, ys, ids, xs, rows_here, tid, [&]() { return w0; }, mult, hj);
+    rowlane_tile<GP, Z, DAMP, COMBINE, false, false>(a, rp, ys, ids, xs, rows_here, tid, [&]() { return w0; }, mult,
+                                                     hj);
     if (use_w0) bias_partial(s_part + stage * 8, mult, hj, tid);
     __syncwarp();
     if (lane == 0) mbar_arrive(empty + stage);
@@ -448,22 +559,28 @@
 }
 
 template <int GP, int Z, bool PROF>
-static HogwildKernelFn pick_d(bool damp, bool combine) {
+static HogwildKernelFn pick_d(bool damp, bool combine, bool dealt) {
+  if (dealt)
+    return combine ? nullptr
+                   : (damp ? fm_sgd_rowlane_kernel<GP, Z, true, false, PROF, true>
+                           : fm_sgd_rowlane_kernel<GP, Z, false, false, PROF, true>);
   if (combine)
-    return damp ? fm_sgd_rowlane_kernel<GP, Z, true, true, PROF> : fm_sgd_rowlane_kernel<GP, Z, false, true, PROF>;
-  return damp ? fm_sgd_rowlane_kernel<GP, Z, true, false, PROF> : fm_sgd_rowlane_kernel<GP, Z, false, false, PROF>;
+    return damp ? fm_sgd_rowlane_kernel<GP, Z, true, true, PROF, false>
+                : fm_sgd_rowlane_kernel<GP, Z, false, true, PROF, false>;
+  return damp ? fm_sgd_rowlane_kernel<GP, Z, true, false, PROF, false>
+              : fm_sgd_rowlane_kernel<GP, Z, false, false, PROF, false>;
 }
 
 template <int GP, int Z>
-static HogwildKernelFn pick_p(bool damp, bool combine, bool prof) {
-  return prof ? pick_d<GP, Z, true>(damp, combine) : pick_d<GP, Z, false>(damp, combine);
+static HogwildKernelFn pick_p(bool damp, bool combine, bool prof, bool dealt) {
+  return prof ? pick_d<GP, Z, true>(damp, combine, dealt) : pick_d<GP, Z, false>(damp, combine, dealt);
 }
 
 template <int GP>
-static HogwildKernelFn pick_z(int z, bool damp, bool combine, bool prof) {
-  if (z <= 1) return pick_p<GP, 1>(damp, combine, prof);
-  if (z <= 2) return pick_p<GP, 2>(damp, combine, prof);
-  if (z <= 4) return pick_p<GP, 4>(damp, combine, prof);
+static HogwildKernelFn pick_z(int z, bool damp, bool combine, bool prof, bool dealt) {
+  if (z <= 1) return pick_p<GP, 1>(damp, combine, prof, dealt);
+  if (z <= 2) return pick_p<GP, 2>(damp, combine, prof, dealt);
+  if (z <= 4) return pick_p<GP, 4>(damp, combine, prof, dealt);
   return nullptr;
 }
 
@@ -488,9 +605,9 @@
   return nullptr;
 }
 
-HogwildKernelFn pick_rowlane_kernel(int gp, int max_row_nnz, bool damp, bool combine, bool prof) {
-  if (gp == 1) return pick_z<1>(max_row_nnz, damp, combine, prof);
-  if (gp == 2) return pick_z<2>(max_row_nnz, damp, combine, prof);
+HogwildKernelFn pick_rowlane_kernel(int gp, int max_row_nnz, bool damp, bool combine, bool prof, bool dealt) {
+  if (gp == 1) return pick_z<1>(max_row_nnz, damp, combine, prof, dealt);
+  if (gp == 2) return pick_z<2>(max_row_nnz, damp, combine, prof, dealt);
   return nullptr;
 }
 
diff --git a/libfm_b200/csrc/fmb200_internal.h b/libfm_b200/csrc/fmb200_internal.h
--- a/libfm_b200/csrc/fmb200_internal.h
+++ b/libfm_b200/csrc/fmb200_internal.h
@@ -61,6 +61,19 @@
 
 constexpr uint64_t kRowSlack = 512 + 8;
 constexpr uint64_t kEntrySlack = 16;
+
+struct RowlaneDeal {
+  DevPtr<uint64_t> row_ptr;
+  DevPtr<uint32_t> col, pos;
+  DevPtr<float> val, target;
+  uint64_t rows_cap = 0, nnz_cap = 0;
+  uint64_t gen = 0;
+  int tr = 0;
+  uint32_t grid = 0;
+  DevPtr<unsigned char> scratch;
+  size_t scratch_bytes = 0;
+  bool matches(uint64_t g, int t, uint32_t G) const { return gen == g && tr == t && grid == G; }
+};
 
 struct DataSlot {
   bool present = false;
@@ -87,6 +100,8 @@
   bool links_ready = false;
   DevPtr<unsigned char> ord_scratch;
   size_t ord_scratch_bytes = 0;
+  RowlaneDeal deal;
+  uint32_t hogwild_epochs = 0;
 };
 
 constexpr int COMM_SEQ_WORD = 0;
@@ -153,6 +168,7 @@
 
 struct EpochConfig {
   int lanes_per_row = 0, slots = 0, rows_per_tile = 0, grid = 0, block = 0, smem = 0, damp = 0;
+  int dealt = 0;
 };
 
 }
@@ -179,6 +195,8 @@
   uint64_t pred_cap = 0;
   fmb::DevPtr<unsigned int> d_sched;
   fmb::DevPtr<unsigned long long> d_acc;
+  fmb::DevPtr<unsigned long long> d_deal_bias;
+  uint64_t deal_bias_cap = 0;
   fmb::DevPtr<unsigned int> d_gbar;
   uint32_t gbar_count = 0;
   fmb::DevPtr<unsigned int> d_flag;
@@ -230,8 +248,10 @@
 bool mcmc_get(const fmb200_ctx* c, double* alpha, double* w_mu, double* w_lambda, double* v_mu, double* v_lambda,
               double* pred_this, double* pred_sum_all, double* pred_sum_all_but5, uint32_t* n_runs);
 cudaError_t launch_sgda_epoch(fmb200_ctx* c, const DataSlot& tr, const DataSlot& va, int lambda_steps);
-cudaError_t launch_sgd_hogwild(fmb200_ctx* c, const DataSlot& d);
+cudaError_t launch_sgd_hogwild(fmb200_ctx* c, DataSlot& d);
 cudaError_t clear_acc_flag(fmb200_ctx* c);
+cudaError_t prepare_rowlane_deal(fmb200_ctx* c, DataSlot& d);
+cudaError_t build_rowlane_deal(fmb200_ctx* c, DataSlot& d, int TR, uint32_t G);
 cudaError_t launch_predict32(fmb200_ctx* c, const DataSlot& d, int transform, double* out_pred,
                              double* partials, int n_blocks);
 cudaError_t launch_p64_to_p32(fmb200_ctx* c);
diff --git a/libfm_b200/model.py b/libfm_b200/model.py
--- a/libfm_b200/model.py
+++ b/libfm_b200/model.py
@@ -426,3 +426,8 @@
         self._check(self.lib.fmb200_last_epoch_config(self._ctx, *[C.byref(x) for x in v]))
         keys = ["lanes_per_row", "slots", "rows_per_tile", "grid", "block", "smem_bytes", "damp"]
         return dict(zip(keys, [x.value for x in v]))
+
+    def epoch_dealt(self) -> bool:
+        v = C.c_int()
+        self._check(self.lib.fmb200_last_epoch_dealt(self._ctx, C.byref(v)))
+        return bool(v.value)
```

Result: faster. 6.634 billion, median of 6 (+11.2%).
